# vinhsuhi/JMAC

Measured on AMD Instinct MI355X. Metric: gnn_layer_edges_per_s, higher is better.
Workload: dtype f32

## Files before the change

include/jmac_hip.h:

```cpp
#ifndef JMAC_HIP_H_
#define JMAC_HIP_H_

#include <stddef.h>
#include <stdint.h>

#ifdef __cplusplus
extern "C" {
#endif

typedef void* jmac_stream_t;

#define JMAC_OK 0
#define JMAC_EINVAL (-1)
#define JMAC_EDIM (-2)
#define JMAC_EWORKSPACE (-3)
#define JMAC_ERANGE (-4)

typedef struct { int32_t seg, beg, end, pslot; } jmac_item_t;
typedef struct { int32_t seg, pslot0, nchunks, pad; } jmac_split_t;

const char* jmac_strerror(int rc);
int jmac_version(void);


// ... 96 lines not shown

size_t jmac_bn_tanh_workspace_bytes(int64_t N, int64_t d);
int jmac_bn_tanh_fwd2_f32(const float* x, int64_t ldx, int64_t N, int64_t d, const float* weight,
                          const float* bias, float* running_mean, float* running_var,
                          int32_t training, float momentum, float eps, float* y, int64_t ldy,
                          float* y2, int64_t ldy2, float* save_mean, float* save_invstd, void* ws,
                          size_t ws_bytes, jmac_stream_t stream);
int jmac_bn_tanh_bwd2_f32(const float* x, int64_t ldx, const float* y, int64_t ldy, const float* gy,
                          int64_t ldgy, const float* gy2, int64_t ldgy2, int64_t N, int64_t d,
                          const float* weight, const float* save_mean, const float* save_invstd,
                          int32_t training, float* gx, int64_t ldgx, float* gweight, float* gbias,
                          void* ws, size_t ws_bytes, jmac_stream_t stream);

#define JMAC_BN_MAX_BLOCKS 16
size_t jmac_bn_tanh_seg_workspace_bytes(int32_t nblocks, int64_t d);
int jmac_bn_tanh_seg_fwd2_f32(const float* x, int64_t ldx, int64_t d, int32_t nblocks, const int64_t* h_blk_ptr,
                              const int32_t* h_order, const float* weight, const float* bias,
                              float* running_mean, float* running_var, float momentum, float eps, float* y,
                              int64_t ldy, float* y2, int64_t ldy2, float* save_mean, float* save_invstd,
                              void* ws, size_t ws_bytes, jmac_stream_t stream);
int jmac_bn_tanh_seg_bwd2_f32(const float* x, int64_t ldx, const float* y, int64_t ldy, const float* gy,
                              int64_t ldgy, const float* gy2, int64_t ldgy2, int64_t d, int32_t nblocks,
                              const int64_t* h_blk_ptr, const float* weight, const float* save_mean,
                              const float* save_invstd, float* gx, int64_t ldgx, float* gweight, float* gbias,
                              void* ws, size_t ws_bytes, jmac_stream_t stream);

int jmac_col_moments_f32(const float* x, int64_t ldx, int64_t N, int64_t d, float* mean, float* m2,
                         void* ws, size_t ws_bytes, jmac_stream_t stream);
int jmac_bn_tanh_apply_f32(const float* x, int64_t ldx, int64_t N, int64_t d, const float* weight,
                           const float* bias, const float* mean, const float* invstd, float* y,
                           int64_t ldy, jmac_stream_t stream);
int jmac_bn_tanh_bwd_sums_f32(const float* x, int64_t ldx, const float* y, int64_t ldy, const float* gy,
                              int64_t ldgy, int64_t N, int64_t d, const float* mean,
                              const float* invstd, float* sums, void* ws, size_t ws_bytes,
                              jmac_stream_t stream);
int jmac_bn_tanh_bwd_apply_f32(const float* x, int64_t ldx, const float* y, int64_t ldy, const float* gy,
                               int64_t ldgy, int64_t N, int64_t d, const float* weight,
                               const float* mean, const float* invstd, const float* sums,
                               int64_t n_total, float* gx, int64_t ldgx, jmac_stream_t stream);

int jmac_row_normalize_fwd_f32(const float* x, int64_t ldx, int64_t N, int64_t d, float eps, float* y,
                               int64_t ldy, float* inv, jmac_stream_t stream);
int jmac_row_normalize_bwd_f32(const float* y, int64_t ldy, const float* g, int64_t ldg, const float* inv,
                               int64_t N, int64_t d, float eps, float* gx, int64_t ldgx,
                               jmac_stream_t stream);

int jmac_row_normalize_drop_fwd_f32(const float* x, int64_t ldx, int64_t N, int64_t d, float eps,
                                    const float* mask, int64_t ldm, float scale, float* y, int64_t ldy,
                                    float* inv, jmac_stream_t stream);
int jmac_row_normalize_drop_bwd_f32(const float* x, int64_t ldx, const float* inv, const float* mask,
                                    int64_t ldm, float scale, const float* g, int64_t ldg, int64_t N,
                                    int64_t d, float eps, float* gx, int64_t ldgx, int32_t accumulate,
                                    jmac_stream_t stream);

int jmac_row_normalize_dropseed_fwd_f32(const float* x, int64_t ldx, int64_t N, int64_t d, float eps,
                                        const int64_t* seed, float p_drop, float* y, int64_t ldy,
                                        float* inv, jmac_stream_t stream);
int jmac_row_normalize_dropseed_bwd_f32(const float* x, int64_t ldx, const float* inv, const int64_t* seed,
                                        float p_drop, const float* g, int64_t ldg, int64_t N, int64_t d,
                                        float eps, float* gx, int64_t ldgx, int32_t accumulate,
                                        jmac_stream_t stream);

int jmac_rows_normalize_dropseed_fwd_f32(const float* x, int64_t ldx, const int64_t* row_map, int64_t N, int64_t d,
                                         float eps, const int64_t* seed, float p_drop, float* x_rows, int64_t ldxr,
                                         float* y, int64_t ldy, float* inv, jmac_stream_t stream);
int jmac_bn_tanh_normalize_dropseed_fwd_f32(const float* x, int64_t ldx, int64_t N, int64_t d, const float* weight,
                                            const float* bias, float* running_mean, float* running_var,
                                            int32_t training, float momentum, float eps, float* y, int64_t ldy,
                                            const int64_t* row_map, float* y_rows, int64_t ldyr, float norm_eps,
                                            const int64_t* seed, float p_drop, float* yn, int64_t ldyn, float* inv,
                                            float* save_mean, float* save_invstd, void* ws, size_t ws_bytes,
                                            jmac_stream_t stream);
int jmac_bn_tanh_bwd_normadj_f32(const float* x, int64_t ldx, const float* y, int64_t ldy, const float* inv,
                                 const float* g, int64_t ldg, float norm_eps, const int64_t* seed, float p_drop,
                                 const float* gy2, int64_t ldgy2, const int64_t* row_map, int64_t N, int64_t d,
                                 const float* weight, const float* save_mean, const float* save_invstd,
                                 int32_t training, float* gx, int64_t ldgx, float* gweight, float* gbias, void* ws,
                                 size_t ws_bytes, jmac_stream_t stream);
int jmac_row_normalize_dropseed_bwd_rows_f32(const float* x, int64_t ldx, const float* inv, const int64_t* seed,
                                             float p_drop, const float* g, int64_t ldg, const float* add,
                                             int64_t ldadd, const int64_t* row_map, int64_t N, int64_t d, float eps,
                                             float* dst, int64_t lddst, int32_t accumulate, jmac_stream_t stream);

int jmac_l1_score_f32(const float* er, int64_t lder, const float* table, int64_t ldt, int64_t B,
                      int64_t N, int64_t d, float* out, int64_t ldout, int32_t accumulate,
                      jmac_stream_t stream);
int jmac_l1_score_bf16(const uint16_t* er, int64_t lder, const uint16_t* table, int64_t ldt, int64_t B,
                       int64_t N, int64_t d, float* out, int64_t ldout, int32_t accumulate,
                       jmac_stream_t stream);

typedef struct {
    const float* ent;  int64_t ld_ent;
    const float* rel;  int64_t ld_rel;
    const void* table; int64_t ld_table;
} jmac_link_layer_t;
size_t jmac_linkpred_rank_workspace_bytes(int64_t B, int64_t d, int32_t n_layers);
int jmac_linkpred_rank_f32(const jmac_link_layer_t* layers, int32_t n_layers, const int32_t* h, const int32_t* r,
                           int32_t pred_head, const int32_t* gold, const int32_t* filt_ptr, const int32_t* filt_idx,
                           int64_t B, int64_t N, int64_t d, int32_t* rank, void* ws, size_t ws_bytes, jmac_stream_t stream);
int jmac_linkpred_rank_bf16(const jmac_link_layer_t* layers, int32_t n_layers, const int32_t* h, const int32_t* r,
                            int32_t pred_head, const int32_t* gold, const int32_t* filt_ptr, const int32_t* filt_idx,
                            int64_t B, int64_t N, int64_t d, int32_t* rank, void* ws, size_t ws_bytes, jmac_stream_t stream);

typedef struct {
    const int64_t* key;
    int64_t        n_keys;
    const int32_t* tail_ptr;
    const int32_t* tail_idx;
} jmac_tail_index_t;

int jmac_linkpred_rank_indexed_f32(const jmac_link_layer_t* layers, int32_t n_layers, const int32_t* h, const int32_t* r,
                                   int32_t pred_head, const int32_t* gold, const jmac_tail_index_t* index, int64_t B,
                                   int64_t N, int64_t d, int32_t* rank, void* ws, size_t ws_bytes, jmac_stream_t stream);
int jmac_linkpred_rank_indexed_bf16(const jmac_link_layer_t* layers, int32_t n_layers, const int32_t* h, const int32_t* r,
                                    int32_t pred_head, const int32_t* gold, const jmac_tail_index_t* index, int64_t B,
                                    int64_t N, int64_t d, int32_t* rank, void* ws, size_t ws_bytes, jmac_stream_t stream);

size_t jmac_linkpred_topk_workspace_bytes(int64_t B, int64_t N, int64_t d, int32_t n_layers, int32_t k);
int jmac_linkpred_topk_f32(const jmac_link_layer_t* layers, int32_t n_layers, const int32_t* h, const int32_t* r,
                           int32_t pred_head, const jmac_tail_index_t* index, int64_t B, int64_t N, int64_t d, int32_t k,
                           float* val, int32_t* idx, void* ws, size_t ws_bytes, jmac_stream_t stream);
int jmac_linkpred_topk_bf16(const jmac_link_layer_t* layers, int32_t n_layers, const int32_t* h, const int32_t* r,
                            int32_t pred_head, const jmac_tail_index_t* index, int64_t B, int64_t N, int64_t d, int32_t k,
                            float* val, int32_t* idx, void* ws, size_t ws_bytes, jmac_stream_t stream);

int jmac_filtered_rank_f32(const float* score, int64_t lds, const int32_t* gold,
                           const int32_t* filt_ptr, const int32_t* filt_idx, int64_t B, int64_t N,
                           int32_t descending, int32_t* rank, jmac_stream_t stream);

int jmac_sim_matrix_f32(const float* A, int64_t lda, const float* B, int64_t ldb, int64_t M,
                        int64_t N, int64_t d, float* C, int64_t ldc, jmac_stream_t stream);

size_t jmac_sim_topk_workspace_bytes(int64_t L, int64_t N, int32_t k);
int jmac_sim_topk_f32(const float* A, int64_t lda, const float* B, int64_t ldb, int64_t L, int64_t N,
                      int64_t d, int32_t k, float* val, int32_t* idx, void* ws, size_t ws_bytes,
                      jmac_stream_t stream);

int jmac_row_topk_f32(const float* S, int64_t lds, int64_t L, int64_t N, int32_t k, float* val,
                      int32_t* idx, jmac_stream_t stream);

size_t jmac_softmax_entropy_workspace_bytes(int64_t n1, int64_t n2);
int jmac_softmax_entropy_f32(const float* A, int64_t lda, const float* B, int64_t ldb, int64_t n1,
                             int64_t n2, int64_t d, float scale, float* ent_rows, float* ent_cols,
                             void* ws, size_t ws_bytes, jmac_stream_t stream);

size_t jmac_sim_softmax_stats_workspace_bytes(int64_t n1, int64_t n2);
int jmac_sim_softmax_stats_f32(const float* A, int64_t lda, const float* B, int64_t ldb, int64_t n1, int64_t n2, int64_t d,
                               float scale, float* row_max, int32_t* row_arg, float* row_sum, float* row_ent, float* col_max,
                               int32_t* col_arg, float* col_sum, float* col_ent, void* ws, size_t ws_bytes,
                               jmac_stream_t stream);

size_t jmac_sim_lse_workspace_bytes(int64_t n1, int64_t n2);
int jmac_sim_lse_f32(const float* A, int64_t lda, const float* B, int64_t ldb, int64_t n1, int64_t n2, int64_t d, float scale,
                     const float* col_add, const float* row_add, float row_shift, float col_shift, float* row_out,
                     float* col_out, void* ws, size_t ws_bytes, jmac_stream_t stream);

int jmac_row_softmax_f32(const float* S, int64_t lds, int64_t n1, int64_t n2, const uint8_t* row_mask,
                         const uint8_t* col_mask, float fill, float scale, float* out, int64_t ldo, float* ent,
                         jmac_stream_t stream);
size_t jmac_col_softmax_workspace_bytes(int64_t n1, int64_t n2);
int jmac_col_softmax_f32(const float* S, int64_t lds, int64_t n1, int64_t n2, const uint8_t* row_mask,
                         const uint8_t* col_mask, float fill, float scale, float* out_t, int64_t ldo, float* ent,
                         void* ws, size_t ws_bytes, jmac_stream_t stream);

size_t jmac_col_topk_workspace_bytes(int64_t n1, int64_t n2, int32_t k);
int jmac_col_topk_f32(const float* S, int64_t lds, int64_t n1, int64_t n2, int32_t k, float* val, void* ws,
                      size_t ws_bytes, jmac_stream_t stream);

int jmac_csls_apply_f32(const float* S, int64_t lds, int64_t n1, int64_t n2, const float* r1,
                        const float* r2, float* out, int64_t ldo, jmac_stream_t stream);

int jmac_csls_rank_f32(const float* S, int64_t lds, int64_t n1, int64_t n2, const float* r1, const float* r2,
                       const int32_t* gold, int32_t* rank, jmac_stream_t stream);

size_t jmac_sim_csls_rank_workspace_bytes(int64_t n1, int64_t n2);
int jmac_sim_csls_rank_f32(const float* A, int64_t lda, const float* B, int64_t ldb, int64_t n1, int64_t n2, int64_t d,
                           const float* r1, const float* r2, const int32_t* gold, int32_t* rank, void* ws, size_t ws_bytes,
                           jmac_stream_t stream);
size_t jmac_sim_csls_topk_workspace_bytes(int64_t n1, int64_t n2, int32_t k);
int jmac_sim_csls_topk_f32(const float* A, int64_t lda, const float* B, int64_t ldb, int64_t n1, int64_t n2, int64_t d,
                           const float* r1, const float* r2, int32_t k, float* val, int32_t* idx, void* ws, size_t ws_bytes,
                           jmac_stream_t stream);
int jmac_sim_csls_topk_viable_f32(const float* A, int64_t lda, const float* B, int64_t ldb, int64_t n1, int64_t n2, int64_t d,
                                  const float* r1, const float* r2, const int32_t* row_id, const uint64_t* best, int32_t k,
                                  float* val, int32_t* idx, void* ws, size_t ws_bytes, jmac_stream_t stream);

size_t jmac_l1_csls_topk_workspace_bytes(int64_t n1, int64_t n2, int64_t d, int32_t k);
int jmac_l1_csls_topk_f32(const float* A, int64_t lda, const float* B, int64_t ldb, int64_t n1, int64_t n2, int64_t d,
                          const float* r1, const float* r2, int32_t k, float* val, int32_t* idx, void* ws, size_t ws_bytes,
                          jmac_stream_t stream);
int jmac_l1_csls_topk_viable_f32(const float* A, int64_t lda, const float* B, int64_t ldb, int64_t n1, int64_t n2, int64_t d,
                                 const float* r1, const float* r2, const int32_t* row_id, const uint64_t* best, int32_t k,
                                 float* val, int32_t* idx, void* ws, size_t ws_bytes, jmac_stream_t stream);
size_t jmac_l1_csls_rank_workspace_bytes(int64_t n1, int64_t n2);
int jmac_l1_csls_rank_f32(const float* A, int64_t lda, const float* B, int64_t ldb, int64_t n1, int64_t n2, int64_t d,
                          const float* r1, const float* r2, const int32_t* gold, int32_t* rank, void* ws, size_t ws_bytes,
                          jmac_stream_t stream);

size_t jmac_stable_match_workspace_bytes(int64_t n1, int64_t n2);
int jmac_stable_match_f32(const int32_t* cand_idx, const float* cand_val, int64_t ld, int64_t n1, int64_t n2, int32_t k, int32_t* ptr,
                          uint64_t* best, int32_t* match1, int32_t* match2, uint64_t* counters, void* ws, size_t ws_bytes,
                          jmac_stream_t stream);

int jmac_gemm_f32(const float* A, int64_t lda, int32_t transA, const float* B, int64_t ldb,
                  int32_t transB, int64_t M, int64_t N, int64_t K, float* C, int64_t ldc,
                  jmac_stream_t stream);

#define JMAC_GEMM_MAX_TASKS 24
#define JMAC_GEMM_ACT_NONE 0
#define JMAC_GEMM_ACT_LEAKY 1
#define JMAC_GEMM_ACT_RELU 2
#define JMAC_GEMM_DACT_LEAKY 3
#define JMAC_GEMM_DACT_RELU 4
typedef struct {
    const float* A;  const float* A2;  int64_t lda;  int64_t a_split;  int32_t transA;  int32_t transB;
    const float* B;  int64_t ldb;
    float* C;  float* C2;  int64_t ldc;  int64_t c_split;
    int64_t M, N, K;
    const float* act_src;  int64_t ld_act_src;
    int32_t act;  int32_t accumulate;  float slope;  int32_t pad_;
} jmac_gemm_task_t;
int jmac_gemm_grouped_f32(const jmac_gemm_task_t* tasks, int32_t n_tasks, jmac_stream_t stream);

#define JMAC_WCAT_MAX 4
int jmac_wcat_pack_seed_f32(const float* const* w_att, const float* const* gcn, float* const* wcat, int32_t n_layers,
                            int64_t d, const float* extra_src, float* extra_dst, int64_t extra_floats,
                            int64_t* const* counters, int32_t n_counters, int64_t* seed_state, int64_t* seed_out,
                            jmac_stream_t stream);
int jmac_wcat_unpack_f32(const float* const* dwcat, float* const* d_watt, float* const* d_gcn,
                         int32_t n_layers, int64_t d, const float* extra_src, float* extra_dst,
                         int64_t extra_floats, jmac_stream_t stream);

#define JMAC_ADAM_MAX_TASKS 64
typedef struct {
    float* p;
    const float* g;
    float* m;
    float* v;
    int64_t n;
    int32_t vec4;
} jmac_adam_task_t;
int jmac_adam_step_f32(const jmac_adam_task_t* tasks, int32_t n_tasks, float* step, double* aux, double lr, double beta1,
                       double beta2, double eps, double weight_decay, int32_t decoupled, int32_t maximize, jmac_stream_t stream);

int jmac_rows_compact_f32(const float* const* h_src, const int64_t* h_ld_src, float* const* h_dst, int32_t n_tables,
                          const int64_t* idx, int64_t n_used, int64_t d, jmac_stream_t stream);
int jmac_rows_expand_f32(const float* const* h_src, float* const* h_dst, const int64_t* h_ld_dst,
                         const int32_t* h_accumulate, int32_t n_tables, const int32_t* pos, int64_t rows, int64_t d,
                         jmac_stream_t stream);


int jmac_triple_l1_fwd_f32(const float* ent, int64_t lde, const float* rel, int64_t ldr,
                           const int64_t* h, const int64_t* r, const int64_t* t, int64_t T,
                           int64_t period, int64_t d, float* score, jmac_stream_t stream);
int jmac_triple_l1_bwd_f32(const float* ent, int64_t lde, const float* rel, int64_t ldr,
                           const int64_t* h, const int64_t* r, const int64_t* t, int64_t T,
                           int64_t period, int64_t d, const float* gscore, float* dent, int64_t ldde, float* drel, int64_t lddr,
                           jmac_stream_t stream);
int jmac_pair_cosine_fwd_stats_f32(const float* e1, int64_t ld1, const float* e2, int64_t ld2, const int64_t* i1,
                                   const int64_t* i2, int64_t L, int64_t d, float* dist, float* stats,
                                   jmac_stream_t stream);
int jmac_pair_cosine_bwd_rows_f32(const float* e1, int64_t ld1, const float* e2, int64_t ld2, int64_t L, int64_t d,
                                  const float* gdist, const float* gscalar, float gscale, const float* stats,
                                  const int32_t* rec, const int32_t* rowptr, int64_t n1, int64_t n2, float* de1,
                                  int64_t ldd1, float* de2, int64_t ldd2, jmac_stream_t stream);

int jmac_triple_l1_margin_bwd_exact2_f32(const float* ent, int64_t lde, const float* rel, int64_t ldr, const int64_t* h,
                                         const int64_t* r, const int64_t* t, int64_t B, int64_t K, int64_t d,
                                         const float* score, const float* gamma, const float* gloss, int64_t ent_off,
                                         int64_t rel_off, float* cnt_ent, float* cnt_rel, float* dent, int64_t rows_ent,
                                         int32_t acc_ent, float* drel, int64_t rows_rel, int32_t acc_rel,
                                         jmac_stream_t stream);

int jmac_triple_l1_margin_fwd_counts_f32(const float* ent, int64_t lde, const float* rel, int64_t ldr, const int64_t* h,
                                         const int64_t* r, const int64_t* t, int64_t B, int64_t K, int64_t d,
                                         const float* gamma, int64_t ent_off, int64_t rel_off, float* cnt_ent,
                                         float* cnt_rel, float* score, jmac_stream_t stream);
int jmac_margin_counts_scale_clear_f32(float* cnt_ent, float* cnt_rel, const float* gloss, int64_t B, int64_t K, int64_t d,
                                       float* dent, int64_t rows_ent, int32_t acc_ent, float* drel, int64_t rows_rel,
                                       int32_t acc_rel, jmac_stream_t stream);

int jmac_vec_mean_acc_f32(const float* x, int64_t n, const float* add_to, float* out, jmac_stream_t stream);

int jmac_pair_cosine_fwd_f32(const float* e1, int64_t ld1, const float* e2, int64_t ld2,
                             const int64_t* i1, const int64_t* i2, int64_t L, int64_t d, float* dist,
                             jmac_stream_t stream);
int jmac_pair_cosine_bwd_f32(const float* e1, int64_t ld1, const float* e2, int64_t ld2,
                             const int64_t* i1, const int64_t* i2, int64_t L, int64_t d,
                             const float* gdist, float* de1, int64_t ldd1, float* de2, int64_t ldd2,
                             jmac_stream_t stream);

int jmac_margin_loss_fwd_acc_f32(const float* score, int64_t B, int64_t K, const float* gamma, const float* add_to,
                                 float* loss, jmac_stream_t stream);
int jmac_margin_loss_bwd_f32(const float* score, int64_t B, int64_t K, const float* gamma,
                             const float* gloss, float* dscore, jmac_stream_t stream);


int jmac_sample_completion_batch(const int64_t* triples, int64_t T, const int64_t* perm, const int32_t* key_of_triple,
                                 const int32_t* tail_ptr, const int32_t* tail_idx, int64_t num_ent, int64_t B, int64_t K,
                                 const int64_t* seed, int64_t* step, int64_t* batch_h, int64_t* batch_r, int64_t* batch_t,
                                 jmac_stream_t stream);

int jmac_scatter_sum_f32(const float* src, const int64_t* index, int64_t E, int64_t d, int64_t N,
                         float* out, jmac_stream_t stream);
size_t jmac_scatter_softmax_workspace_bytes(int64_t N, int64_t d);
int jmac_scatter_softmax_f32(const float* src, const int64_t* index, int64_t E, int64_t d, int64_t N,
                             float* out, void* ws, size_t ws_bytes, jmac_stream_t stream);

#ifdef __cplusplus
}
#endif
#endif
```

jmac_amd/_lib.py:

```python
from __future__ import annotations

import ctypes as C
import os
import re
import weakref
from typing import Optional

_HERE = os.path.dirname(os.path.abspath(__file__))
LIB_PATH = os.environ.get("JMAC_LIB_PATH") or os.path.join(_HERE, "libjmac_hip.so")
HEADER_PATH = os.path.join(os.path.dirname(_HERE), "include", "jmac_hip.h")

_lib: Optional[C.CDLL] = None

i32, i64, f32, vp, sz = C.c_int32, C.c_int64, C.c_float, C.c_void_p, C.c_size_t


class JmacError(RuntimeError):
    pass


class View(C.Structure):
    _fields_ = [("ptr", vp), ("order", vp), ("items", vp), ("splits", vp), ("counts", vp),
                ("n_items_max", i64), ("n_splits_max", i64), ("n_parts_max", i64),
                ("item_edges", vp), ("n_empty", i64), ("n_coop", i64), ("entry_dst", vp)]


class LinkLayer(C.Structure):
    _fields_ = [("ent", vp), ("ld_ent", i64), ("rel", vp), ("ld_rel", i64), ("table", vp), ("ld_table", i64)]


class TailIndex(C.Structure):
    _fields_ = [("key", vp), ("n_keys", i64), ("tail_ptr", vp), ("tail_idx", vp)]


class AggFwdJob(C.Structure):
    _fields_ = [("P", vp), ("ldp", i64), ("QZ", vp), ("ldqz", i64), ("RR", vp), ("ldrr", i64), ("a_att", vp), ("col", vp), ("etype", vp),
                ("by_dst", C.POINTER(View)), ("N", i64), ("d", i64), ("slope", f32), ("loop_rel", i32), ("self_off", i64),
                ("out_scale", f32), ("out", vp), ("ldo", i64), ("seg_max", vp), ("seg_den", vp), ("ws", vp), ("ws_bytes", sz)]


class AdamTask(C.Structure):
    _fields_ = [("p", vp), ("g", vp), ("m", vp), ("v", vp), ("n", i64), ("vec4", i32)]


class GemmTask(C.Structure):
    _fields_ = [("A", vp), ("A2", vp), ("lda", i64), ("a_split", i64), ("transA", i32), ("transB", i32),
                ("B", vp), ("ldb", i64), ("C", vp), ("C2", vp), ("ldc", i64), ("c_split", i64),
                ("M", i64), ("N", i64), ("K", i64), ("act_src", vp), ("ld_act_src", i64),
                ("act", i32), ("accumulate", i32), ("slope", f32), ("pad_", i32)]


_SIGS = {
    "jmac_strerror": (C.c_char_p, [C.c_int]),
    "jmac_version": (C.c_int, []),
    "jmac_graph_workspace_bytes": (sz, [i64, i64]),
    "jmac_index_check": (C.c_int, [vp, i32, i64, i64, i64, vp, vp]),
    "jmac_csr_build": (C.c_int, [vp, vp, i64, i64, i64, vp, vp, vp, vp, vp, sz, vp]),
    "jmac_group_build": (C.c_int, [vp, i64, i64, vp, vp, vp, sz, vp]),
    "jmac_items_max": (i64, [i64, i64, i32, i32]),
    "jmac_splits_max": (i64, [i64, i32, i32]),
    "jmac_parts_max": (i64, [i64, i32, i32]),
    "jmac_items_build": (C.c_int, [vp, i64, i32, i32, i32, vp, vp, vp, vp, sz, vp]),
    "jmac_rel_attn_fwd_workspace_bytes": (sz, [i64, i64]),
    "jmac_item_edges_build": (C.c_int, [vp, vp, i64, vp, vp, vp, vp]),
    "jmac_rel_attn_aggregate_fwd_f32": (C.c_int, [vp, i64, vp, i64, vp, i64, vp, vp, vp, C.POINTER(View),
                                                  i64, i64, f32, i32, i64, f32, vp, i64, vp, vp, vp, sz, vp]),
    "jmac_rel_attn_aggregate_fwd_bf16": (C.c_int, [vp, i64, vp, i64, vp, i64, vp, vp, vp, C.POINTER(View),
                                                   i64, i64, f32, i32, i64, f32, vp, i64, vp, vp, vp, sz, vp]),
    "jmac_rel_attn_aggregate_fwd_bf16_padded": (C.c_int, [vp, i64, vp, i64, vp, i64, i64, vp, vp, vp, C.POINTER(View),
                                                          i64, i64, f32, i32, i64, f32, vp, i64, vp, vp, vp, sz, vp]),
    "jmac_rel_attn_aggregate_fwd_jobs_f32": (C.c_int, [C.POINTER(AggFwdJob), i32, vp]),
    "jmac_softmax_parts_merge_f32": (C.c_int, [vp, i64, vp, vp, vp, i32, i64, i64, vp, i64, vp, f32, vp, i64, vp, vp, vp]),
    "jmac_rel_attn_bwd_workspace_bytes": (sz, [i64, i64, i64, i64, i64, i64, i64, i32]),
    "jmac_rel_attn_aggregate_bwd_f32": (C.c_int, [vp, i64, vp, i64, vp, i64, vp, vp, vp, vp,
                                                  C.POINTER(View), C.POINTER(View), C.POINTER(View),
                                                  i64, i64, i64, i64, i64, f32, i32, i64, f32, vp, i64, vp, vp, vp, i64,
                                                  vp, i64, vp, i64, vp, i64, vp, i32, vp, sz, vp]),
    "jmac_rel_attn_aggregate_bwd_phases_f32": (C.c_int, [vp, i64, vp, i64, vp, i64, vp, vp, vp, vp,
                                                         C.POINTER(View), C.POINTER(View), C.POINTER(View),
                                                         i64, i64, i64, i64, i64, f32, i32, i64, f32, vp, i64, vp, vp, vp, i64,
                                                         vp, i64, vp, i64, vp, i64, vp, i32, vp, sz, vp]),
    "jmac_bn_tanh_workspace_bytes": (sz, [i64, i64]),
    "jmac_bn_tanh_fwd2_f32": (C.c_int, [vp, i64, i64, i64, vp, vp, vp, vp, i32, f32, f32, vp, i64, vp, i64, vp, vp,
                                        vp, sz, vp]),
    "jmac_bn_tanh_bwd2_f32": (C.c_int, [vp, i64, vp, i64, vp, i64, vp, i64, i64, i64, vp, vp, vp, i32, vp, i64, vp, vp,
                                        vp, sz, vp]),
    "jmac_bn_tanh_seg_workspace_bytes": (sz, [i32, i64]),
    "jmac_bn_tanh_seg_fwd2_f32": (C.c_int, [vp, i64, i64, i32, C.POINTER(i64), C.POINTER(i32), vp, vp, vp, vp, f32, f32, vp, i64,
                                            vp, i64, vp, vp, vp, sz, vp]),
    "jmac_bn_tanh_seg_bwd2_f32": (C.c_int, [vp, i64, vp, i64, vp, i64, vp, i64, i64, i32, C.POINTER(i64), vp, vp, vp, vp, i64,
                                            vp, vp, vp, sz, vp]),
    "jmac_row_normalize_drop_fwd_f32": (C.c_int, [vp, i64, i64, i64, f32, vp, i64, f32, vp, i64, vp, vp]),
    "jmac_row_normalize_drop_bwd_f32": (C.c_int, [vp, i64, vp, vp, i64, f32, vp, i64, i64, i64, f32, vp, i64, i32, vp]),
    "jmac_row_normalize_dropseed_fwd_f32": (C.c_int, [vp, i64, i64, i64, f32, vp, f32, vp, i64, vp, vp]),
    "jmac_row_normalize_dropseed_bwd_f32": (C.c_int, [vp, i64, vp, vp, f32, vp, i64, i64, i64, f32, vp, i64, i32, vp]),
    "jmac_rows_normalize_dropseed_fwd_f32": (C.c_int, [vp, i64, vp, i64, i64, f32, vp, f32, vp, i64, vp, i64, vp, vp]),
    "jmac_bn_tanh_normalize_dropseed_fwd_f32": (C.c_int, [vp, i64, i64, i64, vp, vp, vp, vp, i32, f32, f32, vp, i64, vp, vp, i64,
                                                          f32, vp, f32, vp, i64, vp, vp, vp, vp, sz, vp]),
    "jmac_bn_tanh_bwd_normadj_f32": (C.c_int, [vp, i64, vp, i64, vp, vp, i64, f32, vp, f32, vp, i64, vp, i64, i64, vp, vp, vp,
                                               i32, vp, i64, vp, vp, vp, sz, vp]),
    "jmac_row_normalize_dropseed_bwd_rows_f32": (C.c_int, [vp, i64, vp, vp, f32, vp, i64, vp, i64, vp, i64, i64, f32, vp, i64,
                                                           i32, vp]),
    "jmac_gemm_grouped_f32": (C.c_int, [C.POINTER(GemmTask), i32, vp]),
    "jmac_wcat_pack_seed_f32": (C.c_int, [C.POINTER(vp), C.POINTER(vp), C.POINTER(vp), i32, i64, vp, vp, i64, C.POINTER(vp), i32, vp, vp, vp]),
    "jmac_adam_step_f32": (C.c_int, [C.POINTER(AdamTask), i32, vp, vp, C.c_double, C.c_double, C.c_double, C.c_double, C.c_double, i32, i32,
                                     vp]),
    "jmac_wcat_unpack_f32": (C.c_int, [C.POINTER(vp), C.POINTER(vp), C.POINTER(vp), i32, i64, vp, vp, i64, vp]),
    "jmac_rows_compact_f32": (C.c_int, [C.POINTER(vp), C.POINTER(i64), C.POINTER(vp), i32, vp, i64, i64, vp]),
    "jmac_rows_expand_f32": (C.c_int, [C.POINTER(vp), C.POINTER(vp), C.POINTER(i64), C.POINTER(i32), i32, vp, i64, i64, vp]),
    "jmac_col_moments_f32": (C.c_int, [vp, i64, i64, i64, vp, vp, vp, sz, vp]),
    "jmac_bn_tanh_apply_f32": (C.c_int, [vp, i64, i64, i64, vp, vp, vp, vp, vp, i64, vp]),
    "jmac_bn_tanh_bwd_sums_f32": (C.c_int, [vp, i64, vp, i64, vp, i64, i64, i64, vp, vp, vp, vp, sz, vp]),
    "jmac_bn_tanh_bwd_apply_f32": (C.c_int, [vp, i64, vp, i64, vp, i64, i64, i64, vp, vp, vp, vp, i64, vp, i64, vp]),
    "jmac_row_normalize_fwd_f32": (C.c_int, [vp, i64, i64, i64, f32, vp, i64, vp, vp]),
    "jmac_row_normalize_bwd_f32": (C.c_int, [vp, i64, vp, i64, vp, i64, i64, f32, vp, i64, vp]),
    "jmac_l1_score_f32": (C.c_int, [vp, i64, vp, i64, i64, i64, i64, vp, i64, i32, vp]),
    "jmac_l1_score_bf16": (C.c_int, [vp, i64, vp, i64, i64, i64, i64, vp, i64, i32, vp]),
    "jmac_filtered_rank_f32": (C.c_int, [vp, i64, vp, vp, vp, i64, i64, i32, vp, vp]),
    "jmac_linkpred_rank_workspace_bytes": (sz, [i64, i64, i32]),
    "jmac_linkpred_rank_f32": (C.c_int, [vp, i32, vp, vp, i32, vp, vp, vp, i64, i64, i64, vp, vp, sz, vp]),
    "jmac_linkpred_rank_bf16": (C.c_int, [vp, i32, vp, vp, i32, vp, vp, vp, i64, i64, i64, vp, vp, sz, vp]),
    "jmac_linkpred_rank_indexed_f32": (C.c_int, [vp, i32, vp, vp, i32, vp, vp, i64, i64, i64, vp, vp, sz, vp]),
    "jmac_linkpred_rank_indexed_bf16": (C.c_int, [vp, i32, vp, vp, i32, vp, vp, i64, i64, i64, vp, vp, sz, vp]),
    "jmac_linkpred_topk_workspace_bytes": (sz, [i64, i64, i64, i32, i32]),
    "jmac_linkpred_topk_f32": (C.c_int, [vp, i32, vp, vp, i32, vp, i64, i64, i64, i32, vp, vp, vp, sz, vp]),
    "jmac_linkpred_topk_bf16": (C.c_int, [vp, i32, vp, vp, i32, vp, i64, i64, i64, i32, vp, vp, vp, sz, vp]),
    "jmac_sim_matrix_f32": (C.c_int, [vp, i64, vp, i64, i64, i64, i64, vp, i64, vp]),
    "jmac_sim_topk_workspace_bytes": (sz, [i64, i64, i32]),
    "jmac_sim_topk_f32": (C.c_int, [vp, i64, vp, i64, i64, i64, i64, i32, vp, vp, vp, sz, vp]),
    "jmac_col_topk_workspace_bytes": (sz, [i64, i64, i32]),
    "jmac_col_topk_f32": (C.c_int, [vp, i64, i64, i64, i32, vp, vp, sz, vp]),
    "jmac_row_topk_f32": (C.c_int, [vp, i64, i64, i64, i32, vp, vp, vp]),
    "jmac_softmax_entropy_workspace_bytes": (sz, [i64, i64]),
    "jmac_softmax_entropy_f32": (C.c_int, [vp, i64, vp, i64, i64, i64, i64, f32, vp, vp, vp, sz, vp]),
    "jmac_sim_softmax_stats_workspace_bytes": (sz, [i64, i64]),
    "jmac_sim_softmax_stats_f32": (C.c_int, [vp, i64, vp, i64, i64, i64, i64, f32, vp, vp, vp, vp, vp, vp, vp, vp, vp, sz, vp]),
    "jmac_sim_lse_workspace_bytes": (sz, [i64, i64]),
    "jmac_sim_lse_f32": (C.c_int, [vp, i64, vp, i64, i64, i64, i64, f32, vp, vp, f32, f32, vp, vp, vp, sz, vp]),
    "jmac_row_softmax_f32": (C.c_int, [vp, i64, i64, i64, vp, vp, f32, f32, vp, i64, vp, vp]),
    "jmac_col_softmax_workspace_bytes": (sz, [i64, i64]),
    "jmac_col_softmax_f32": (C.c_int, [vp, i64, i64, i64, vp, vp, f32, f32, vp, i64, vp, vp, sz, vp]),
    "jmac_csls_rank_f32": (C.c_int, [vp, i64, i64, i64, vp, vp, vp, vp, vp]),
    "jmac_csls_apply_f32": (C.c_int, [vp, i64, i64, i64, vp, vp, vp, i64, vp]),
    "jmac_sim_csls_rank_workspace_bytes": (sz, [i64, i64]),
    "jmac_sim_csls_rank_f32": (C.c_int, [vp, i64, vp, i64, i64, i64, i64, vp, vp, vp, vp, vp, sz, vp]),
    "jmac_sim_csls_topk_workspace_bytes": (sz, [i64, i64, i32]),
    "jmac_sim_csls_topk_f32": (C.c_int, [vp, i64, vp, i64, i64, i64, i64, vp, vp, i32, vp, vp, vp, sz, vp]),
    "jmac_sim_csls_topk_viable_f32": (C.c_int, [vp, i64, vp, i64, i64, i64, i64, vp, vp, vp, vp, i32, vp, vp, vp, sz, vp]),
    "jmac_l1_csls_topk_workspace_bytes": (sz, [i64, i64, i64, i32]),
    "jmac_l1_csls_topk_f32": (C.c_int, [vp, i64, vp, i64, i64, i64, i64, vp, vp, i32, vp, vp, vp, sz, vp]),
    "jmac_l1_csls_topk_viable_f32": (C.c_int, [vp, i64, vp, i64, i64, i64, i64, vp, vp, vp, vp, i32, vp, vp, vp, sz, vp]),
    "jmac_l1_csls_rank_workspace_bytes": (sz, [i64, i64]),
    "jmac_l1_csls_rank_f32": (C.c_int, [vp, i64, vp, i64, i64, i64, i64, vp, vp, vp, vp, vp, sz, vp]),
    "jmac_stable_match_workspace_bytes": (sz, [i64, i64]),
    "jmac_stable_match_f32": (C.c_int, [vp, vp, i64, i64, i64, i32, vp, vp, vp, vp, vp, vp, sz, vp]),
    "jmac_gemm_f32": (C.c_int, [vp, i64, i32, vp, i64, i32, i64, i64, i64, vp, i64, vp]),
    "jmac_triple_l1_fwd_f32": (C.c_int, [vp, i64, vp, i64, vp, vp, vp, i64, i64, i64, vp, vp]),
    "jmac_triple_l1_bwd_f32": (C.c_int, [vp, i64, vp, i64, vp, vp, vp, i64, i64, i64, vp, vp, i64, vp, i64, vp]),
    "jmac_pair_cosine_fwd_stats_f32": (C.c_int, [vp, i64, vp, i64, vp, vp, i64, i64, vp, vp, vp]),
    "jmac_pair_cosine_fwd_f32": (C.c_int, [vp, i64, vp, i64, vp, vp, i64, i64, vp, vp]),
    "jmac_pair_cosine_bwd_f32": (C.c_int, [vp, i64, vp, i64, vp, vp, i64, i64, vp, vp, i64, vp, i64, vp]),
    "jmac_pair_cosine_bwd_rows_f32": (C.c_int, [vp, i64, vp, i64, i64, i64, vp, vp, f32, vp, vp, vp, i64, i64, vp, i64, vp, i64, vp]),
    "jmac_triple_l1_margin_bwd_exact2_f32": (C.c_int, [vp, i64, vp, i64, vp, vp, vp, i64, i64, i64, vp, vp, vp, i64, i64, vp, vp,
                                                       vp, i64, i32, vp, i64, i32, vp]),
    "jmac_triple_l1_margin_fwd_counts_f32": (C.c_int, [vp, i64, vp, i64, vp, vp, vp, i64, i64, i64, vp, i64, i64, vp, vp, vp, vp]),
    "jmac_margin_counts_scale_clear_f32": (C.c_int, [vp, vp, vp, i64, i64, i64, vp, i64, i32, vp, i64, i32, vp]),
    "jmac_vec_mean_acc_f32": (C.c_int, [vp, i64, vp, vp, vp]),
    "jmac_margin_loss_fwd_acc_f32": (C.c_int, [vp, i64, i64, vp, vp, vp, vp]),
    "jmac_margin_loss_bwd_f32": (C.c_int, [vp, i64, i64, vp, vp, vp, vp]),
    "jmac_sample_completion_batch": (C.c_int, [vp, i64, vp, vp, vp, vp, i64, i64, i64, vp, vp, vp, vp, vp, vp]),
    "jmac_scatter_sum_f32": (C.c_int, [vp, vp, i64, i64, i64, vp, vp]),
    "jmac_scatter_softmax_workspace_bytes": (sz, [i64, i64]),
    "jmac_scatter_softmax_f32": (C.c_int, [vp, vp, i64, i64, i64, vp, vp, sz, vp]),
}


_TESTING_SIGS = {
    "jmac_rel_attn_aggregate_fwd_lanes64_f32": _SIGS["jmac_rel_attn_aggregate_fwd_f32"],
    "jmac_rel_attn_aggregate_fwd_lanes64_bf16_padded": _SIGS["jmac_rel_attn_aggregate_fwd_bf16_padded"],
    "jmac_gemm_nt_x3_f32": (C.c_int, [vp, i64, vp, i64, i64, i64, i64, vp, i64, vp]),
}


def header_text(path: str = HEADER_PATH) -> str:
    return re.sub(r"/\*.*?\*/", "", open(path).read(), flags=re.S)


# ... 122 lines not shown
```

jmac_amd/csrc/norm.hip:

```cpp
#include <initializer_list>

#include "common.h"

using namespace jmac;

namespace {

constexpr int kBlock = 256;
constexpr int kStatBlocks = 512;

__global__ __launch_bounds__(kBlock) void col_stats_partial_kernel(const float* __restrict__ x, int64_t ldx, int64_t N,
                                                                   int D4, float* __restrict__ partial) {
    extern __shared__ __attribute__((aligned(16))) char smem[];
    float4* red = reinterpret_cast<float4*>(smem);
    const int rpb = kBlock / D4 > 0 ? kBlock / D4 : 1;
    const int tid = threadIdx.x;
    for (int cbase = 0; cbase < D4; cbase += kBlock) {
        const int rsub = D4 >= kBlock ? 0 : tid / D4;
        const int c4 = D4 >= kBlock ? cbase + tid : tid % D4;
        const bool active = (D4 >= kBlock ? c4 < D4 : tid < rpb * D4);
        float4 s1 = f4zero(), s2 = f4zero();
        if (active) {
            const float4 K = ld4(x + c4 * 4);
            for (int64_t r = (int64_t)blockIdx.x * rpb + rsub; r < N; r += (int64_t)gridDim.x * rpb) {
                float4 v = ld4(x + r * ldx + c4 * 4);
                v.x -= K.x; v.y -= K.y; v.z -= K.z; v.w -= K.w;
                s1.x += v.x; s1.y += v.y; s1.z += v.z; s1.w += v.w;
                s2.x = fmaf(v.x, v.x, s2.x); s2.y = fmaf(v.y, v.y, s2.y); s2.z = fmaf(v.z, v.z, s2.z); s2.w = fmaf(v.w, v.w, s2.w);
            }
        }
        if (D4 >= kBlock) {
            if (active) {
                st4(partial + ((int64_t)blockIdx.x * 2 + 0) * D4 * 4 + c4 * 4, s1);
                st4(partial + ((int64_t)blockIdx.x * 2 + 1) * D4 * 4 + c4 * 4, s2);
            }
        } else {
            if (active) {
                red[(0 * rpb + rsub) * D4 + c4] = s1;
                red[(1 * rpb + rsub) * D4 + c4] = s2;
            }
            __syncthreads();
            if (tid < D4) {
                float4 a1 = red[tid], a2 = red[rpb * D4 + tid];
                for (int q = 1; q < rpb; ++q) {
                    float4 b1 = red[q * D4 + tid], b2 = red[(rpb + q) * D4 + tid];
                    a1.x += b1.x; a1.y += b1.y; a1.z += b1.z; a1.w += b1.w;
                    a2.x += b2.x; a2.y += b2.y; a2.z += b2.z; a2.w += b2.w;
                }
                st4(partial + ((int64_t)blockIdx.x * 2 + 0) * D4 * 4 + tid * 4, a1);
                st4(partial + ((int64_t)blockIdx.x * 2 + 1) * D4 * 4 + tid * 4, a2);
            }
            break;
        }
    }
}

__global__ void bn_finalize_kernel(const float* __restrict__ sums, const float* __restrict__ x, int64_t N,
                                   int d, float eps, float momentum, float* __restrict__ running_mean,
                                   float* __restrict__ running_var, float* __restrict__ save_mean,
                                   float* __restrict__ save_invstd) {
    const int c = blockIdx.x * blockDim.x + threadIdx.x;
    if (c >= d) return;
    const float s1 = sums[c], s2 = sums[d + c];
    const float n = (float)N;
    const float K = x[c];
    const float mshift = s1 / n;
    const float mean = K + mshift;
    float var = s2 / n - mshift * mshift;
    var = var > 0.f ? var : 0.f;
    save_mean[c] = mean;
    save_invstd[c] = rsqrtf(var + eps);
    if (running_mean) running_mean[c] = (1.f - momentum) * running_mean[c] + momentum * mean;
    if (running_var) {
        const float unbiased = N > 1 ? var * n / (n - 1.f) : var;
        running_var[c] = (1.f - momentum) * running_var[c] + momentum * unbiased;
    }
}

constexpr int RF_COLS = 16, RF_LANES = 1024 / RF_COLS;
__global__ __launch_bounds__(1024) void bn_reduce_finalize_kernel(const float* __restrict__ partial, int nparts,
                                                                  const float* __restrict__ x, int64_t N, int d, float eps,
                                                                  float momentum, float* __restrict__ running_mean,
                                                                  float* __restrict__ running_var, float* __restrict__ save_mean,
                                                                  float* __restrict__ save_invstd) {
    __shared__ float red1[RF_LANES][RF_COLS], red2[RF_LANES][RF_COLS];
    const int cl = threadIdx.x % RF_COLS, rl = threadIdx.x / RF_COLS;
    const int c = blockIdx.x * RF_COLS + cl;
    float a1 = 0.f, a2 = 0.f, b1 = 0.f, b2 = 0.f;
    if (c < d) {
        int p = rl;
        for (; p + RF_LANES < nparts; p += 2 * RF_LANES) {
            a1 += partial[(int64_t)p * 2 * d + c];
            a2 += partial[(int64_t)p * 2 * d + d + c];
            b1 += partial[(int64_t)(p + RF_LANES) * 2 * d + c];
            b2 += partial[(int64_t)(p + RF_LANES) * 2 * d + d + c];
        }
        if (p < nparts) {
            a1 += partial[(int64_t)p * 2 * d + c];
            a2 += partial[(int64_t)p * 2 * d + d + c];
        }
    }
    red1[rl][cl] = a1 + b1;
    red2[rl][cl] = a2 + b2;
    __syncthreads();
    if (rl == 0 && c < d) {
        float s1 = red1[0][cl], s2 = red2[0][cl];
#pragma unroll 8
        for (int r = 1; r < RF_LANES; ++r) {
            s1 += red1[r][cl];
            s2 += red2[r][cl];
        }
        const float n = (float)N;
        const float mshift = s1 / n;
        const float mean = x[c] + mshift;
        float var = s2 / n - mshift * mshift;
        var = var > 0.f ? var : 0.f;
        save_mean[c] = mean;
        save_invstd[c] = rsqrtf(var + eps);
        if (running_mean) running_mean[c] = (1.f - momentum) * running_mean[c] + momentum * mean;
        if (running_var) {
            const float unbiased = N > 1 ? var * n / (n - 1.f) : var;
            running_var[c] = (1.f - momentum) * running_var[c] + momentum * unbiased;
        }
    }
}

__global__ void moments_finalize_kernel(const float* __restrict__ sums, const float* __restrict__ x, int64_t N, int d,
                                        float* __restrict__ mean, float* __restrict__ m2) {
    const int c = blockIdx.x * blockDim.x + threadIdx.x;
    if (c >= d) return;
    const float s1 = sums[c], s2 = sums[d + c], n = (float)N;
    mean[c] = x[c] + s1 / n;
    const float v = s2 - s1 * s1 / n;
    m2[c] = v > 0.f ? v : 0.f;
}

__global__ void bn_eval_stats_kernel(const float* __restrict__ running_mean, const float* __restrict__ running_var, int d,
                                     float eps, float* __restrict__ save_mean, float* __restrict__ save_invstd) {
    const int c = blockIdx.x * blockDim.x + threadIdx.x;
    if (c < d) {
        save_mean[c] = running_mean[c];
        save_invstd[c] = rsqrtf(running_var[c] + eps);
    }
}

__global__ __launch_bounds__(kBlock) void bn_tanh_apply_kernel(const float* __restrict__ x, int64_t ldx, int64_t N, int D4,
                                                               const float* __restrict__ weight, const float* __restrict__ bias,
                                                               const float* __restrict__ mean, const float* __restrict__ invstd,
                                                               float* __restrict__ y, int64_t ldy, float* __restrict__ y2,
                                                               int64_t ldy2) {
    const int64_t total = N * D4;
    for (int64_t i = (int64_t)blockIdx.x * kBlock + threadIdx.x; i < total; i += (int64_t)gridDim.x * kBlock) {
        const int64_t r = i / D4;
        const int c4 = (int)(i % D4);
        const float4 v = ld4(x + r * ldx + c4 * 4);
        const float4 mu = ld4(mean + c4 * 4), is = ld4(invstd + c4 * 4), w = ld4(weight + c4 * 4), b = ld4(bias + c4 * 4);
        float4 o;
        o.x = tanhf(fmaf((v.x - mu.x) * is.x, w.x, b.x));
        o.y = tanhf(fmaf((v.y - mu.y) * is.y, w.y, b.y));
        o.z = tanhf(fmaf((v.z - mu.z) * is.z, w.z, b.z));
        o.w = tanhf(fmaf((v.w - mu.w) * is.w, w.w, b.w));
        st4(y + r * ldy + c4 * 4, o);
        if (y2) st4(y2 + r * ldy2 + c4 * 4, o);
    }
}

__global__ __launch_bounds__(kBlock) void bn_bwd_partial_kernel(const float* __restrict__ x, int64_t ldx,
                                                                const float* __restrict__ y, int64_t ldy,
                                                                const float* __restrict__ gy, int64_t ldgy,
                                                                const float* __restrict__ gy2, int64_t ldgy2, int64_t N, int D4,
                                                                const float* __restrict__ mean, const float* __restrict__ invstd,
                                                                float* __restrict__ partial) {
    extern __shared__ __attribute__((aligned(16))) char smem[];
    float4* red = reinterpret_cast<float4*>(smem);
    const int rpb = kBlock / D4 > 0 ? kBlock / D4 : 1;
    const int tid = threadIdx.x;
    for (int cbase = 0; cbase < D4; cbase += kBlock) {
        const int rsub = D4 >= kBlock ? 0 : tid / D4;
        const int c4 = D4 >= kBlock ? cbase + tid : tid % D4;
        const bool active = (D4 >= kBlock ? c4 < D4 : tid < rpb * D4);
        float4 s1 = f4zero(), s2 = f4zero();
        if (active) {
            const float4 mu = ld4(mean + c4 * 4), is = ld4(invstd + c4 * 4);
            for (int64_t r = (int64_t)blockIdx.x * rpb + rsub; r < N; r += (int64_t)gridDim.x * rpb) {
                const float4 xv = ld4(x + r * ldx + c4 * 4), yv = ld4(y + r * ldy + c4 * 4);
                float4 g = ld4(gy + r * ldgy + c4 * 4);
                if (gy2) {
                    const float4 g2 = ld4(gy2 + r * ldgy2 + c4 * 4);
                    g.x += g2.x; g.y += g2.y; g.z += g2.z; g.w += g2.w;
                }
                const float gz0 = g.x * (1.f - yv.x * yv.x), gz1 = g.y * (1.f - yv.y * yv.y);
                const float gz2 = g.z * (1.f - yv.z * yv.z), gz3 = g.w * (1.f - yv.w * yv.w);
                s1.x += gz0; s1.y += gz1; s1.z += gz2; s1.w += gz3;
                s2.x = fmaf(gz0, (xv.x - mu.x) * is.x, s2.x); s2.y = fmaf(gz1, (xv.y - mu.y) * is.y, s2.y);
                s2.z = fmaf(gz2, (xv.z - mu.z) * is.z, s2.z); s2.w = fmaf(gz3, (xv.w - mu.w) * is.w, s2.w);
            }
        }
        if (D4 >= kBlock) {
            if (active) {
                st4(partial + ((int64_t)blockIdx.x * 2 + 0) * D4 * 4 + c4 * 4, s1);
                st4(partial + ((int64_t)blockIdx.x * 2 + 1) * D4 * 4 + c4 * 4, s2);
            }
        } else {
            if (active) {
                red[(0 * rpb + rsub) * D4 + c4] = s1;
                red[(1 * rpb + rsub) * D4 + c4] = s2;
            }
// ... 940 lines not shown
#pragma unroll
            for (int k = 0; k < 2; ++k) {
                const int c = (ok[k] ? cc[k] : 0) * 4;
                xv[u][k] = ld4(x + row[u] * ldx + c);
                yv[u][k] = ld4(y + row[u] * ldy + c);
                q[u][k] = ld4(g + row[u] * ldg + c);
                if (gy2) g2[u][k] = ld4(gy2 + s[u] * ldgy2 + c);
            }
        }
        normalize_drop_adjoint_rows<SEED, ROWFORM, R>(ds, key, row, D4, cc, ok, eps, iv, yv, q);
#pragma unroll
        for (int u = 0; u < R; ++u) {
            if (r0 + u >= N) break;
#pragma unroll
            for (int k = 0; k < 2; ++k) {
                if (!ok[k]) continue;
                float4 gg = adjoint_scale(iv[u], q[u][k]);
                if (gy2) gg = add4(gg, g2[u][k]);
                const float4 yy = yv[u][k], xx = xv[u][k];
                float4 o;
#define JMAC_BN_BWD(comp)                                                                                                       \
                o.comp = bn_bwd_apply_elem(gg.comp, yy.comp, xx.comp, mu[k].comp, is[k].comp, w[k].comp, gw[k].comp, gb[k].comp, \
                                           training, invn);
                JMAC_BN_BWD(x) JMAC_BN_BWD(y) JMAC_BN_BWD(z) JMAC_BN_BWD(w)
#undef JMAC_BN_BWD
                st4(gx + (r0 + u) * ldgx + cc[k] * 4, o);
            }
        }
    }
}

template <bool SEED, bool ROWFORM, int R>
__global__ __launch_bounds__(kBlock) void row_normalize_drop_bwd_scatter_kernel(const float* __restrict__ x, int64_t ldx,
                                                                                const float* __restrict__ inv, DropSrc ds,
                                                                                const float* __restrict__ g, int64_t ldg,
                                                                                const float* __restrict__ add, int64_t ldadd,
                                                                                const int64_t* __restrict__ map, int64_t N, int D4,
                                                                                float eps, float* __restrict__ dst, int64_t lddst,
                                                                                int accumulate) {
    const int lane = lane_id();
    const int64_t w0 = (int64_t)blockIdx.x * (kBlock / 64) + (threadIdx.x >> 6), nw = (int64_t)gridDim.x * (kBlock / 64);
    const uint2 key = drop_key(ds, SEED);
    const int cc[2] = {lane, lane + 64};
    const bool ok[2] = {cc[0] < D4, cc[1] < D4};
    for (int64_t r0 = w0 * R; r0 < N; r0 += nw * R) {
        float4 v[R][2], q[R][2], p[R][2], old[R][2];
        float iv[R];
        int64_t row[R], s[R];
#pragma unroll
        for (int u = 0; u < R; ++u) {
            row[u] = r0 + u < N ? r0 + u : N - 1;
            s[u] = map ? map[row[u]] : row[u];
        }
#pragma unroll
        for (int u = 0; u < R; ++u) {
            iv[u] = inv[row[u]];
#pragma unroll
            for (int k = 0; k < 2; ++k) {
                const int c = (ok[k] ? cc[k] : 0) * 4;
                v[u][k] = ld4(x + row[u] * ldx + c);
                q[u][k] = ld4(g + row[u] * ldg + c);
                if (add) p[u][k] = ld4(add + row[u] * ldadd + c);
                if (accumulate) old[u][k] = ld4(dst + s[u] * lddst + c);
            }
        }
        normalize_drop_adjoint_rows<SEED, ROWFORM, R>(ds, key, row, D4, cc, ok, eps, iv, v, q);
#pragma unroll
        for (int u = 0; u < R; ++u) {
            if (r0 + u >= N) break;
#pragma unroll
            for (int k = 0; k < 2; ++k) {
                if (!ok[k]) continue;
                float4 o = add ? adjoint_scale_add<ROWFORM>(iv[u], q[u][k], p[u][k]) : adjoint_scale(iv[u], q[u][k]);
                if (accumulate) o = add4(o, old[u][k]);
                st4(dst + s[u] * lddst + cc[k] * 4, o);
            }
        }
    }
}

constexpr int kDropRows = 4;
constexpr int64_t kDropRowsMinN = 2048;

}

extern "C" {

size_t jmac_bn_tanh_workspace_bytes(int64_t N, int64_t d) {
    (void)N;
    return align_up((size_t)(kStatBlocks + 1) * 2 * (d > 0 ? d : 0) * 4) + 256;
}

int jmac_bn_tanh_fwd2_f32(const float* x, int64_t ldx, int64_t N, int64_t d, const float* weight, const float* bias,
                          float* running_mean, float* running_var, int32_t training, float momentum, float eps, float* y,
                          int64_t ldy, float* y2, int64_t ldy2, float* save_mean, float* save_invstd, void* ws, size_t ws_bytes,
                          jmac_stream_t stream) {
    if (N < 0 || !weight || !bias || !save_mean || !save_invstd) return JMAC_EINVAL;
    if (d <= 0 || d % 4 || ldx % 4 || ldy % 4 || (y2 && ldy2 % 4)) return JMAC_EDIM;
    if (N == 0) return JMAC_OK;
    if (!x || !y) return JMAC_EINVAL;
    hipStream_t st = (hipStream_t)stream;
    const int D4 = (int)(d / 4);
    if (training) {
        if (!ws || ws_bytes < jmac_bn_tanh_workspace_bytes(N, d)) return JMAC_EWORKSPACE;
        float* partial = (float*)ws;
        const unsigned g = stat_grid(N, D4);
        hipLaunchKernelGGL(col_stats_partial_kernel, dim3(g), dim3(kBlock), stat_smem(D4), st, x, ldx, N, D4, partial);
        hipLaunchKernelGGL(bn_reduce_finalize_kernel, dim3((unsigned)((d + RF_COLS - 1) / RF_COLS)), dim3(1024), 0, st, partial,
                           (int)g, x, N, (int)d, eps, momentum, running_mean, running_var, save_mean, save_invstd);
    } else {
        if (!running_mean || !running_var) return JMAC_EINVAL;
        hipLaunchKernelGGL(bn_eval_stats_kernel, dim3((unsigned)((d + 255) / 256)), dim3(256), 0, st, running_mean, running_var,
                           (int)d, eps, save_mean, save_invstd);
    }
    hipLaunchKernelGGL(bn_tanh_apply_kernel, dim3(stream_grid(N * D4)), dim3(kBlock), 0, st, x, ldx, N, D4, weight, bias,
                       save_mean, save_invstd, y, ldy, y2, ldy2);
    return (int)hipGetLastError();
}

int jmac_bn_tanh_bwd2_f32(const float* x, int64_t ldx, const float* y, int64_t ldy, const float* gy, int64_t ldgy,
                          const float* gy2, int64_t ldgy2, int64_t N, int64_t d, const float* weight, const float* save_mean,
                          const float* save_invstd, int32_t training, float* gx, int64_t ldgx, float* gweight, float* gbias,
                          void* ws, size_t ws_bytes, jmac_stream_t stream) {
    if (N < 0 || !weight || !save_mean || !save_invstd || !gweight || !gbias) return JMAC_EINVAL;
    if (d <= 0 || d % 4 || ldx % 4 || ldy % 4 || ldgy % 4 || ldgx % 4 || (gy2 && ldgy2 % 4)) return JMAC_EDIM;
    if (!ws || ws_bytes < jmac_bn_tanh_workspace_bytes(N, d)) return JMAC_EWORKSPACE;
    hipStream_t st = (hipStream_t)stream;
    const int D4 = (int)(d / 4);
    float* partial = (float*)ws;
    unsigned g = 0;
    if (N > 0) {
        if (!x || !y || !gy || !gx) return JMAC_EINVAL;
        g = stat_grid(N, D4);
        hipLaunchKernelGGL(bn_bwd_partial_kernel, dim3(g), dim3(kBlock), stat_smem(D4), st, x, ldx, y, ldy, gy, ldgy, gy2, ldgy2, N,
                           D4, save_mean, save_invstd, partial);
    }
    if (gweight == gbias + d) {
        launch_reduce_rows(partial, (int)g, (int)(2 * d), 1.f, gbias, st);
    } else {
        float* sums = partial + (size_t)kStatBlocks * 2 * d;
        launch_reduce_rows(partial, (int)g, (int)(2 * d), 1.f, sums, st);
        hipLaunchKernelGGL(bn_bwd_finalize_kernel, dim3((unsigned)((d + 255) / 256)), dim3(256), 0, st, sums, (int)d, gweight, gbias);
    }
    if (N > 0)
        hipLaunchKernelGGL(bn_bwd_apply_kernel, dim3(stream_grid(N * D4)), dim3(kBlock), 0, st, x, ldx, y, ldy, gy, ldgy, gy2, ldgy2, N,
                           D4, weight, save_mean, save_invstd, gweight, gbias, training, 1.f / (float)N, gx, ldgx);
    return (int)hipGetLastError();
}

int jmac_row_normalize_fwd_f32(const float* x, int64_t ldx, int64_t N, int64_t d, float eps, float* y, int64_t ldy, float* inv,
                               jmac_stream_t stream) {
    if (N < 0 || d <= 0 || d >= INT32_MAX) return JMAC_EINVAL;
    if (N == 0) return JMAC_OK;
    if (!x || !y || !inv) return JMAC_EINVAL;
    int64_t blocks = (N + kBlock / 64 - 1) / (kBlock / 64);
    if (blocks > 8192) blocks = 8192;
    hipLaunchKernelGGL(row_normalize_fwd_kernel, dim3((unsigned)blocks), dim3(kBlock), 0, (hipStream_t)stream, x, ldx, N, (int)d, eps,
                       y, ldy, inv);
    return (int)hipGetLastError();
}

int jmac_row_normalize_bwd_f32(const float* y, int64_t ldy, const float* g, int64_t ldg, const float* inv, int64_t N, int64_t d,
                               float eps, float* gx, int64_t ldgx, jmac_stream_t stream) {
    if (N < 0 || d <= 0 || d >= INT32_MAX) return JMAC_EINVAL;
    if (N == 0) return JMAC_OK;
    if (!y || !g || !inv || !gx) return JMAC_EINVAL;
    int64_t blocks = (N + kBlock / 64 - 1) / (kBlock / 64);
    if (blocks > 8192) blocks = 8192;
    hipLaunchKernelGGL(row_normalize_bwd_kernel, dim3((unsigned)blocks), dim3(kBlock), 0, (hipStream_t)stream, y, ldy, g, ldg, inv, N,
                       (int)d, eps, gx, ldgx);
    return (int)hipGetLastError();
}

static int drop_fwd(const float* x, int64_t ldx, int64_t N, int64_t d, float eps, const DropSrc& ds, bool seeded, float* y, int64_t ldy,
                    float* inv, jmac_stream_t stream) {
    if (N < 0 || d <= 0 || d >= INT32_MAX) return JMAC_EINVAL;
    if (d % 4 || ldx % 4 || ldy % 4 || (ds.mask && ds.ldm % 4)) return JMAC_EDIM;
    if (N == 0) return JMAC_OK;
    if (!x || !y || !inv) return JMAC_EINVAL;
    if ((((uintptr_t)x | (uintptr_t)y | (uintptr_t)ds.mask) & 15) != 0) return JMAC_EDIM;
    if (d <= 512 && N >= kDropRowsMinN) {
        int64_t rb = ((N + kDropRows - 1) / kDropRows + kBlock / 64 - 1) / (kBlock / 64);
        if (rb > 8192) rb = 8192;
        if (seeded)
            hipLaunchKernelGGL((row_normalize_drop_fwd_rows_kernel<true, kDropRows>), dim3((unsigned)rb), dim3(kBlock), 0,
                               (hipStream_t)stream, x, ldx, N, (int)(d / 4), eps, ds, y, ldy, inv);
        else
            hipLaunchKernelGGL((row_normalize_drop_fwd_rows_kernel<false, kDropRows>), dim3((unsigned)rb), dim3(kBlock), 0,
                               (hipStream_t)stream, x, ldx, N, (int)(d / 4), eps, ds, y, ldy, inv);
        return (int)hipGetLastError();
    }
    int64_t blocks = (N + kBlock / 64 - 1) / (kBlock / 64);
    if (blocks > 8192) blocks = 8192;
    if (seeded)
        hipLaunchKernelGGL(row_normalize_drop_fwd_kernel<true>, dim3((unsigned)blocks), dim3(kBlock), 0, (hipStream_t)stream, x, ldx, N,
                           (int)(d / 4), eps, ds, y, ldy, inv);
    else
        hipLaunchKernelGGL(row_normalize_drop_fwd_kernel<false>, dim3((unsigned)blocks), dim3(kBlock), 0, (hipStream_t)stream, x, ldx, N,
                           (int)(d / 4), eps, ds, y, ldy, inv);
    return (int)hipGetLastError();
}

static int drop_bwd(const float* x, int64_t ldx, const float* inv, const DropSrc& ds, bool seeded, const float* g, int64_t ldg, int64_t N,
                    int64_t d, float eps, float* gx, int64_t ldgx, int32_t accumulate, jmac_stream_t stream) {
    if (N < 0 || d <= 0 || d >= INT32_MAX) return JMAC_EINVAL;
    if (d % 4 || ldx % 4 || ldg % 4 || ldgx % 4 || (ds.mask && ds.ldm % 4)) return JMAC_EDIM;
    if (N == 0) return JMAC_OK;
    if (!x || !inv || !g || !gx) return JMAC_EINVAL;
    if ((((uintptr_t)x | (uintptr_t)g | (uintptr_t)gx | (uintptr_t)ds.mask) & 15) != 0) return JMAC_EDIM;
    if (d <= 512 && N >= kDropRowsMinN) {
        int64_t rb = ((N + kDropRows - 1) / kDropRows + kBlock / 64 - 1) / (kBlock / 64);
        if (rb > 8192) rb = 8192;
        if (seeded)
            hipLaunchKernelGGL((row_normalize_drop_bwd_rows_kernel<true, kDropRows>), dim3((unsigned)rb), dim3(kBlock), 0,
                               (hipStream_t)stream, x, ldx, inv, ds, g, ldg, N, (int)(d / 4), eps, gx, ldgx, accumulate ? 1 : 0);
        else
            hipLaunchKernelGGL((row_normalize_drop_bwd_rows_kernel<false, kDropRows>), dim3((unsigned)rb), dim3(kBlock), 0,
                               (hipStream_t)stream, x, ldx, inv, ds, g, ldg, N, (int)(d / 4), eps, gx, ldgx, accumulate ? 1 : 0);
        return (int)hipGetLastError();
    }
    int64_t blocks = (N + kBlock / 64 - 1) / (kBlock / 64);
    if (blocks > 8192) blocks = 8192;
    if (seeded)
        hipLaunchKernelGGL(row_normalize_drop_bwd_kernel<true>, dim3((unsigned)blocks), dim3(kBlock), 0, (hipStream_t)stream, x, ldx, inv,
                           ds, g, ldg, N, (int)(d / 4), eps, gx, ldgx, accumulate ? 1 : 0);
    else
        hipLaunchKernelGGL(row_normalize_drop_bwd_kernel<false>, dim3((unsigned)blocks), dim3(kBlock), 0, (hipStream_t)stream, x, ldx, inv,
                           ds, g, ldg, N, (int)(d / 4), eps, gx, ldgx, accumulate ? 1 : 0);
    return (int)hipGetLastError();
}

static int seeded_src(const int64_t* seed, float p_drop, DropSrc& ds) {
    if (!seed || !(p_drop >= 0.f) || !(p_drop < 1.f)) return JMAC_EINVAL;
    const double keep = 1.0 - (double)p_drop, t = keep * 4294967296.0;
    ds = DropSrc{nullptr, 0, seed, t >= 4294967295.0 ? 0xFFFFFFFFu : (uint32_t)t, (float)(1.0 / keep)};
    return JMAC_OK;
}

int jmac_row_normalize_drop_fwd_f32(const float* x, int64_t ldx, int64_t N, int64_t d, float eps, const float* mask, int64_t ldm,
                                    float scale, float* y, int64_t ldy, float* inv, jmac_stream_t stream) {
    return drop_fwd(x, ldx, N, d, eps, DropSrc{mask, ldm, nullptr, 0u, scale}, false, y, ldy, inv, stream);
}

int jmac_row_normalize_drop_bwd_f32(const float* x, int64_t ldx, const float* inv, const float* mask, int64_t ldm, float scale,
                                    const float* g, int64_t ldg, int64_t N, int64_t d, float eps, float* gx, int64_t ldgx,
                                    int32_t accumulate, jmac_stream_t stream) {
    return drop_bwd(x, ldx, inv, DropSrc{mask, ldm, nullptr, 0u, scale}, false, g, ldg, N, d, eps, gx, ldgx, accumulate, stream);
}

int jmac_row_normalize_dropseed_fwd_f32(const float* x, int64_t ldx, int64_t N, int64_t d, float eps, const int64_t* seed,
                                        float p_drop, float* y, int64_t ldy, float* inv, jmac_stream_t stream) {
    DropSrc ds;
    if (int rc = seeded_src(seed, p_drop, ds)) return rc;
    return drop_fwd(x, ldx, N, d, eps, ds, true, y, ldy, inv, stream);
}

int jmac_row_normalize_dropseed_bwd_f32(const float* x, int64_t ldx, const float* inv, const int64_t* seed, float p_drop,
                                        const float* g, int64_t ldg, int64_t N, int64_t d, float eps, float* gx, int64_t ldgx,
                                        int32_t accumulate, jmac_stream_t stream) {
    DropSrc ds;
    if (int rc = seeded_src(seed, p_drop, ds)) return rc;
    return drop_bwd(x, ldx, inv, ds, true, g, ldg, N, d, eps, gx, ldgx, accumulate, stream);
}

static int fused_src(const int64_t* seed, float p_drop, DropSrc& ds) {
    if (seed) return seeded_src(seed, p_drop, ds);
    ds = DropSrc{nullptr, 0, nullptr, 0u, 1.f};
    return JMAC_OK;
}
static bool aligned16(std::initializer_list<const void*> ps) {
    uintptr_t a = 0;
    for (const void* p : ps) a |= (uintptr_t)p;
    return (a & 15) == 0;
}
static unsigned rows_grid(int64_t N, int R) {
    int64_t rb = ((N + R - 1) / R + kBlock / 64 - 1) / (kBlock / 64);
    return (unsigned)(rb > 8192 ? 8192 : rb);
}
#define JMAC_LAUNCH_SEEDED(kernel, R, grid, st, ...)                                                                      \
    do {                                                                                                                  \
        if (ds.seed) hipLaunchKernelGGL((kernel<true, R>), dim3(grid), dim3(kBlock), 0, st, __VA_ARGS__);                 \
        else hipLaunchKernelGGL((kernel<false, R>), dim3(grid), dim3(kBlock), 0, st, __VA_ARGS__);                        \
    } while (0)
#define JMAC_LAUNCH_ADJ(kernel, R, grid, st, ...)                                                                         \
    do {                                                                                                                  \
        const bool rowform = N >= kDropRowsMinN;                                                                          \
        if (ds.seed && rowform) hipLaunchKernelGGL((kernel<true, true, R>), dim3(grid), dim3(kBlock), 0, st, __VA_ARGS__); \
        else if (ds.seed) hipLaunchKernelGGL((kernel<true, false, R>), dim3(grid), dim3(kBlock), 0, st, __VA_ARGS__);     \
        else if (rowform) hipLaunchKernelGGL((kernel<false, true, R>), dim3(grid), dim3(kBlock), 0, st, __VA_ARGS__);     \
        else hipLaunchKernelGGL((kernel<false, false, R>), dim3(grid), dim3(kBlock), 0, st, __VA_ARGS__);                 \
    } while (0)

int jmac_rows_normalize_dropseed_fwd_f32(const float* x, int64_t ldx, const int64_t* row_map, int64_t N, int64_t d, float eps,
                                         const int64_t* seed, float p_drop, float* x_rows, int64_t ldxr, float* y, int64_t ldy,
                                         float* inv, jmac_stream_t stream) {
    DropSrc ds;
    if (int rc = fused_src(seed, p_drop, ds)) return rc;
    if (N < 0) return JMAC_EINVAL;
    if (d <= 0 || d > 512 || d % 4 || ldx % 4 || ldy % 4 || (x_rows && ldxr % 4)) return JMAC_EDIM;
    if (N == 0) return JMAC_OK;
    if (!x || !y || !inv) return JMAC_EINVAL;
    if (!aligned16({x, y, x_rows})) return JMAC_EDIM;
    JMAC_LAUNCH_SEEDED(rows_normalize_drop_fwd_kernel, kFuseRows, rows_grid(N, kFuseRows), (hipStream_t)stream, x, ldx, row_map, N,
                       (int)(d / 4), eps, ds, x_rows, ldxr, y, ldy, inv);
    return (int)hipGetLastError();
}

int jmac_bn_tanh_normalize_dropseed_fwd_f32(const float* x, int64_t ldx, int64_t N, int64_t d, const float* weight, const float* bias,
                                            float* running_mean, float* running_var, int32_t training, float momentum, float eps,
                                            float* y, int64_t ldy, const int64_t* row_map, float* y_rows, int64_t ldyr, float norm_eps,
                                            const int64_t* seed, float p_drop, float* yn, int64_t ldyn, float* inv, float* save_mean,
                                            float* save_invstd, void* ws, size_t ws_bytes, jmac_stream_t stream) {
    DropSrc ds;
    if (int rc = fused_src(seed, p_drop, ds)) return rc;
    if (N < 0 || !weight || !bias || !save_mean || !save_invstd || (row_map == nullptr) != (y_rows == nullptr)) return JMAC_EINVAL;
    if (d <= 0 || d > 512 || d % 4 || ldx % 4 || ldy % 4 || ldyn % 4 || (y_rows && ldyr % 4)) return JMAC_EDIM;
    if (N == 0) return JMAC_OK;
    if (!x || !y || !yn || !inv) return JMAC_EINVAL;
    if (!aligned16({x, y, y_rows, yn, weight, bias, save_mean, save_invstd})) return JMAC_EDIM;
    hipStream_t st = (hipStream_t)stream;
    const int D4 = (int)(d / 4);
    if (training) {
        if (!ws || ws_bytes < jmac_bn_tanh_workspace_bytes(N, d)) return JMAC_EWORKSPACE;
        float* partial = (float*)ws;
        const unsigned g = stat_grid(N, D4);
        hipLaunchKernelGGL(col_stats_partial_kernel, dim3(g), dim3(kBlock), stat_smem(D4), st, x, ldx, N, D4, partial);
        hipLaunchKernelGGL(bn_reduce_finalize_kernel, dim3((unsigned)((d + RF_COLS - 1) / RF_COLS)), dim3(1024), 0, st, partial,
                           (int)g, x, N, (int)d, eps, momentum, running_mean, running_var, save_mean, save_invstd);
    } else {
        if (!running_mean || !running_var) return JMAC_EINVAL;
        hipLaunchKernelGGL(bn_eval_stats_kernel, dim3((unsigned)((d + 255) / 256)), dim3(256), 0, st, running_mean, running_var,
                           (int)d, eps, save_mean, save_invstd);
    }
    JMAC_LAUNCH_SEEDED(bn_tanh_normalize_drop_fwd_kernel, kFuseRows, rows_grid(N, kFuseRows), st, x, ldx, N, D4, weight, bias,
                       (const float*)save_mean, (const float*)save_invstd, y, ldy, row_map, y_rows, ldyr, norm_eps, ds, yn, ldyn, inv);
    return (int)hipGetLastError();
}

int jmac_bn_tanh_bwd_normadj_f32(const float* x, int64_t ldx, const float* y, int64_t ldy, const float* inv, const float* g,
                                 int64_t ldg, float norm_eps, const int64_t* seed, float p_drop, const float* gy2, int64_t ldgy2,
                                 const int64_t* row_map, int64_t N, int64_t d, const float* weight, const float* save_mean,
                                 const float* save_invstd, int32_t training, float* gx, int64_t ldgx, float* gweight, float* gbias,
                                 void* ws, size_t ws_bytes, jmac_stream_t stream) {
    DropSrc ds;
    if (int rc = fused_src(seed, p_drop, ds)) return rc;
    if (N < 0 || !weight || !save_mean || !save_invstd || !gweight || !gbias) return JMAC_EINVAL;
    if (d <= 0 || d > 512 || d % 4 || ldx % 4 || ldy % 4 || ldg % 4 || ldgx % 4 || (gy2 && ldgy2 % 4)) return JMAC_EDIM;
    if (!ws || ws_bytes < jmac_bn_tanh_workspace_bytes(N, d)) return JMAC_EWORKSPACE;
    if (!aligned16({x, y, g, gy2, gx, weight, save_mean, save_invstd, gweight, gbias, ws})) return JMAC_EDIM;
    hipStream_t st = (hipStream_t)stream;
    const int D4 = (int)(d / 4);
    float* partial = (float*)ws;
    unsigned pg = 0;
    if (N > 0) {
        if (!x || !y || !inv || !g || !gx) return JMAC_EINVAL;
        pg = stat_grid(N, D4);
        const int rpb = kBlock / D4;
        const unsigned threads = 64u * (unsigned)(rpb < kBlock / 64 ? rpb : kBlock / 64);
        const bool rowform = N >= kDropRowsMinN;
#define JMAC_PARTIAL(SD, RF)                                                                                                      \
        hipLaunchKernelGGL((bn_bwd_partial_adj_kernel<SD, RF, kFuseBwdRows>), dim3(pg), dim3(threads), stat_smem(D4), st, x, ldx, \
                           y, ldy, g, ldg, inv, ds, norm_eps, gy2, ldgy2, row_map, N, D4, save_mean, save_invstd, partial)
        if (ds.seed && rowform) JMAC_PARTIAL(true, true);
        else if (ds.seed) JMAC_PARTIAL(true, false);
        else if (rowform) JMAC_PARTIAL(false, true);
        else JMAC_PARTIAL(false, false);
#undef JMAC_PARTIAL
    }
    if (gweight == gbias + d) {
        launch_reduce_rows(partial, (int)pg, (int)(2 * d), 1.f, gbias, st);
    } else {
        float* sums = partial + (size_t)kStatBlocks * 2 * d;
        launch_reduce_rows(partial, (int)pg, (int)(2 * d), 1.f, sums, st);
        hipLaunchKernelGGL(bn_bwd_finalize_kernel, dim3((unsigned)((d + 255) / 256)), dim3(256), 0, st, sums, (int)d, gweight, gbias);
    }
    if (N > 0)
        JMAC_LAUNCH_ADJ(bn_bwd_apply_adj_kernel, kFuseBwdRows, rows_grid(N, kFuseBwdRows), st, x, ldx, y, ldy, g, ldg, inv, ds,
                           norm_eps, gy2, ldgy2, row_map, N, D4, weight, save_mean, save_invstd, (const float*)gweight,
                           (const float*)gbias, training ? 1 : 0, 1.f / (float)N, gx, ldgx);
    return (int)hipGetLastError();
}

int jmac_row_normalize_dropseed_bwd_rows_f32(const float* x, int64_t ldx, const float* inv, const int64_t* seed, float p_drop,
                                             const float* g, int64_t ldg, const float* add, int64_t ldadd, const int64_t* row_map,
                                             int64_t N, int64_t d, float eps, float* dst, int64_t lddst, int32_t accumulate,
                                             jmac_stream_t stream) {
    DropSrc ds;
    if (int rc = fused_src(seed, p_drop, ds)) return rc;
    if (N < 0) return JMAC_EINVAL;
    if (d <= 0 || d > 512 || d % 4 || ldx % 4 || ldg % 4 || lddst % 4 || (add && ldadd % 4)) return JMAC_EDIM;
    if (N == 0) return JMAC_OK;
    if (!x || !inv || !g || !dst) return JMAC_EINVAL;
    if (!aligned16({x, g, add, dst})) return JMAC_EDIM;
    JMAC_LAUNCH_ADJ(row_normalize_drop_bwd_scatter_kernel, kFuseBwdRows, rows_grid(N, kFuseBwdRows), (hipStream_t)stream, x, ldx,
                       inv, ds, g, ldg, add, ldadd, row_map, N, (int)(d / 4), eps, dst, lddst, accumulate ? 1 : 0);
    return (int)hipGetLastError();
}
#undef JMAC_LAUNCH_SEEDED
#undef JMAC_LAUNCH_ADJ

static int make_seg(int32_t nblocks, const int64_t* blk_ptr, const int32_t* order, int D4, SegTab& s) {
    if (nblocks < 1 || nblocks > kMaxSeg || !blk_ptr || blk_ptr[0] != 0) return JMAC_EINVAL;
    s.nb = nblocks;
    unsigned seen = 0;
    s.gofs[0] = 0;
    for (int b = 0; b < kMaxSeg; ++b) s.order[b] = 0;
    for (int b = 0; b < nblocks; ++b) {
        const int64_t n = blk_ptr[b + 1] - blk_ptr[b];
        if (n <= 0) return JMAC_EINVAL;
        s.ptr[b] = blk_ptr[b];
        s.gofs[b + 1] = s.gofs[b] + (int)stat_grid(n, D4);
        const int o = order ? order[b] : b;
        if (o < 0 || o >= nblocks || (seen >> o & 1u)) return JMAC_EINVAL;
        seen |= 1u << o;
        s.order[b] = o;
    }
    for (int b = nblocks; b <= kMaxSeg; ++b) s.ptr[b] = blk_ptr[nblocks];
    for (int b = nblocks + 1; b <= kMaxSeg; ++b) s.gofs[b] = s.gofs[nblocks];
    return JMAC_OK;
// ... 116 lines not shown
```

jmac_amd/csrc/optim.hip:

```cpp
#include "common.h"

namespace {

constexpr int kAdamBlock = 256;

struct AdamArgs {
    jmac_adam_task_t t[JMAC_ADAM_MAX_TASKS];
    int chunk_end[JMAC_ADAM_MAX_TASKS];
    int n_tasks, n_chunks;
    double lr, beta1, beta2, eps, weight_decay;
    int decoupled, maximize, advance;
    float* step;
    double* aux;
};

struct AdamConst {
    float one_minus_b1, b2, one_minus_b2, step_size, inv_bc2_sqrt, eps, wd, lr_wd;
};

__device__ __forceinline__ void adam_elem(float& p, float g, float& m, float& v, const AdamConst& c, bool decoupled, bool maximize) {
    if (maximize) g = -g;
    if (c.wd != 0.f) {
        if (decoupled) p = p - c.lr_wd * p;
        else g = g + c.wd * p;
    }
    m = m + (g - m) * c.one_minus_b1;
    v = v * c.b2 + c.one_minus_b2 * g * g;
    const float denom = __fsqrt_rn(v) * c.inv_bc2_sqrt + c.eps;
    p = p - c.step_size * (m / denom);
}

template <int V>
__global__ __launch_bounds__(kAdamBlock) void adam_step_kernel(const AdamArgs a) {
    constexpr int kChunk = kAdamBlock * 4 * V;
    const int ch = blockIdx.x;
    int task = 0;
    if (a.n_chunks > 0) {
        int lo = 0, hi = a.n_tasks - 1;
        while (lo < hi) {
            const int mid = (lo + hi) >> 1;
            if (ch >= a.chunk_end[mid]) lo = mid + 1; else hi = mid;
        }
        task = lo;
    }
    const jmac_adam_task_t T = a.t[task];
    const int first = task ? a.chunk_end[task - 1] : 0;
    const int64_t base = (int64_t)(ch - first) * kChunk;
    const int64_t left = a.n_chunks > 0 ? T.n - base : 0;
    const bool full = left >= kChunk && T.vec4;
    float4 p[V], g[V], m[V], v[V];
    if (full) {
        const float4* p4 = reinterpret_cast<const float4*>(T.p + base);
        const float4* g4 = reinterpret_cast<const float4*>(T.g + base);
        const float4* m4 = reinterpret_cast<const float4*>(T.m + base);
        const float4* v4 = reinterpret_cast<const float4*>(T.v + base);
#pragma unroll
        for (int u = 0; u < V; ++u) {
            const int i = threadIdx.x + u * kAdamBlock;
            p[u] = p4[i]; g[u] = g4[i]; m[u] = m4[i]; v[u] = v4[i];
        }
    }
    AdamConst c;
    {
        const double bc1 = 1.0 - a.aux[0] * a.beta1, bc2 = 1.0 - a.aux[1] * a.beta2;
        c.one_minus_b1 = (float)(1.0 - a.beta1);
        c.b2 = (float)a.beta2;
        c.one_minus_b2 = (float)(1.0 - a.beta2);
        c.step_size = (float)(a.lr / bc1);
        c.inv_bc2_sqrt = (float)(1.0 / sqrt(bc2));
        c.eps = (float)a.eps;
        c.wd = (float)a.weight_decay;
        c.lr_wd = (float)(a.lr * a.weight_decay);
    }
    const bool dec = a.decoupled != 0, mx = a.maximize != 0;
    if (full) {
        float4* p4 = reinterpret_cast<float4*>(T.p + base);
        float4* m4 = reinterpret_cast<float4*>(T.m + base);
        float4* v4 = reinterpret_cast<float4*>(T.v + base);
#pragma unroll
        for (int u = 0; u < V; ++u) {
            adam_elem(p[u].x, g[u].x, m[u].x, v[u].x, c, dec, mx);
            adam_elem(p[u].y, g[u].y, m[u].y, v[u].y, c, dec, mx);
            adam_elem(p[u].z, g[u].z, m[u].z, v[u].z, c, dec, mx);
            adam_elem(p[u].w, g[u].w, m[u].w, v[u].w, c, dec, mx);
        }
#pragma unroll
        for (int u = 0; u < V; ++u) {
            const int i = threadIdx.x + u * kAdamBlock;
            p4[i] = p[u]; m4[i] = m[u]; v4[i] = v[u];
        }
    } else {
        const int64_t n = left < kChunk ? left : kChunk;
        for (int64_t i = threadIdx.x; i < n; i += kAdamBlock) {
            float pp = T.p[base + i], mm = T.m[base + i], vv = T.v[base + i];
            adam_elem(pp, T.g[base + i], mm, vv, c, dec, mx);
            T.p[base + i] = pp; T.m[base + i] = mm; T.v[base + i] = vv;
        }
    }
    if (a.advance) {
        __syncthreads();
        if (threadIdx.x == 0) {
            unsigned int* ticket = reinterpret_cast<unsigned int*>(a.aux + 2);
            const unsigned int done = __hip_atomic_fetch_add(ticket, 1u, __ATOMIC_RELAXED, __HIP_MEMORY_SCOPE_AGENT);
            if (done == gridDim.x - 1) {
                a.step[0] = a.step[0] + 1.f;
                a.aux[0] = a.aux[0] * a.beta1;
                a.aux[1] = a.aux[1] * a.beta2;
                __hip_atomic_store(ticket, 0u, __ATOMIC_RELAXED, __HIP_MEMORY_SCOPE_AGENT);
            }
        }
    }
}

template <int V>
int launch_adam(const jmac_adam_task_t* tasks, int32_t n_tasks, float* step, double* aux, double lr, double beta1, double beta2,
                double eps, double weight_decay, int32_t decoupled, int32_t maximize, hipStream_t st) {
    constexpr int kChunk = kAdamBlock * 4 * V;
    int32_t at = 0;
    do {
        AdamArgs a;
        const int32_t n = (n_tasks - at) < JMAC_ADAM_MAX_TASKS ? (n_tasks - at) : JMAC_ADAM_MAX_TASKS;
        int64_t chunks = 0;
        for (int32_t i = 0; i < n; ++i) {
            const jmac_adam_task_t& t = tasks[at + i];
            if (t.n < 0 || (t.n > 0 && (!t.p || !t.g || !t.m || !t.v))) return JMAC_EINVAL;
            a.t[i] = t;
            a.t[i].vec4 = !(((uintptr_t)t.p | (uintptr_t)t.g | (uintptr_t)t.m | (uintptr_t)t.v) & 15);
            chunks += (t.n + kChunk - 1) / kChunk;
            if (chunks >= INT32_MAX) return JMAC_ERANGE;
            a.chunk_end[i] = (int)chunks;
        }
        for (int32_t i = n; i < JMAC_ADAM_MAX_TASKS; ++i) {
            a.t[i] = jmac_adam_task_t{nullptr, nullptr, nullptr, nullptr, 0, 0};
            a.chunk_end[i] = INT32_MAX;
        }
        a.n_tasks = n > 0 ? n : 1;
        a.n_chunks = (int)chunks;
        a.lr = lr; a.beta1 = beta1; a.beta2 = beta2; a.eps = eps; a.weight_decay = weight_decay;
        a.decoupled = decoupled; a.maximize = maximize;
        at += n;
        a.advance = at >= n_tasks;
        a.step = step;
        a.aux = aux;
        hipLaunchKernelGGL(adam_step_kernel<V>, dim3((unsigned)(chunks < 1 ? 1 : chunks)), dim3(kAdamBlock), 0, st, a);
        const int rc = (int)hipGetLastError();
        if (rc) return rc;
    } while (at < n_tasks);
    return JMAC_OK;
}

}

extern "C" int jmac_adam_step_f32(const jmac_adam_task_t* tasks, int32_t n_tasks, float* step, double* aux, double lr, double beta1,
                                  double beta2, double eps, double weight_decay, int32_t decoupled, int32_t maximize,
                                  jmac_stream_t stream) {
    if (n_tasks < 0 || !step || !aux || ((uintptr_t)aux & 7) || (n_tasks > 0 && !tasks)) return JMAC_EINVAL;
    if (!(lr >= 0.0) || !(eps >= 0.0) || !(beta1 >= 0.0 && beta1 < 1.0) || !(beta2 >= 0.0 && beta2 < 1.0) || !(weight_decay >= 0.0))
        return JMAC_EINVAL;
    for (int32_t i = 0; i < n_tasks; ++i)
        if (tasks[i].n < 0 || (tasks[i].n > 0 && (!tasks[i].p || !tasks[i].g || !tasks[i].m || !tasks[i].v))) return JMAC_EINVAL;
    return launch_adam<4>(tasks, n_tasks, step, aux, lr, beta1, beta2, eps, weight_decay, decoupled, maximize, (hipStream_t)stream);
}
```

jmac_amd/csrc/scatter.hip:

```cpp
#include "common.h"

using namespace jmac;

namespace {

__device__ __forceinline__ void atomic_max_f32(float* addr, float v) {
    if (v >= 0.f) atomicMax(reinterpret_cast<int*>(addr), __float_as_int(v));
    else atomicMin(reinterpret_cast<unsigned int*>(addr), __float_as_uint(v));
}

__global__ void scatter_sum_kernel(const float* __restrict__ src, const int64_t* __restrict__ index, int64_t E, int64_t d,
                                   int64_t N, float* __restrict__ out) {
    const int64_t total = E * d;
    for (int64_t i = (int64_t)blockIdx.x * blockDim.x + threadIdx.x; i < total; i += (int64_t)gridDim.x * blockDim.x) {
        const int64_t e = i / d, c = i % d;
        const int64_t r = index[e];
        if (r >= 0 && r < N) atomicAdd(out + r * d + c, src[i]);
    }
}

__global__ void fill_f32_kernel(float* __restrict__ p, int64_t n, float v) {
    for (int64_t i = (int64_t)blockIdx.x * blockDim.x + threadIdx.x; i < n; i += (int64_t)gridDim.x * blockDim.x) p[i] = v;
}

// ... 5 lines not shown
        const int64_t r = index[e];
        if (r >= 0 && r < N) atomic_max_f32(mx + r * d + c, src[i]);
    }
}

__global__ void seg_expsum_kernel(const float* __restrict__ src, const int64_t* __restrict__ index, int64_t E, int64_t d,
                                  int64_t N, const float* __restrict__ mx, float* __restrict__ sum, float* __restrict__ out) {
    const int64_t total = E * d;
    for (int64_t i = (int64_t)blockIdx.x * blockDim.x + threadIdx.x; i < total; i += (int64_t)gridDim.x * blockDim.x) {
        const int64_t e = i / d, c = i % d;
        const int64_t r = index[e];
        if (r >= 0 && r < N) {
            const float ex = expf(src[i] - mx[r * d + c]);
            out[i] = ex;
            atomicAdd(sum + r * d + c, ex);
        }
    }
}

__global__ void seg_div_kernel(const int64_t* __restrict__ index, int64_t E, int64_t d, int64_t N,
                               const float* __restrict__ sum, float* __restrict__ out) {
    const int64_t total = E * d;
    for (int64_t i = (int64_t)blockIdx.x * blockDim.x + threadIdx.x; i < total; i += (int64_t)gridDim.x * blockDim.x) {
        const int64_t e = i / d, c = i % d;
        const int64_t r = index[e];
        if (r >= 0 && r < N) out[i] = out[i] / sum[r * d + c];
    }
}

inline unsigned grid_for(int64_t total) {
    int64_t g = (total + 255) / 256;
    if (g < 1) g = 1;
    return (unsigned)(g < 16384 ? g : 16384);
}

}

extern "C" {

int jmac_scatter_sum_f32(const float* src, const int64_t* index, int64_t E, int64_t d, int64_t N, float* out,
                         jmac_stream_t stream) {
    if (E < 0 || d <= 0 || N < 0) return JMAC_EINVAL;
    if (E == 0) return JMAC_OK;
    if (!src || !index || !out) return JMAC_EINVAL;
    hipLaunchKernelGGL(scatter_sum_kernel, dim3(grid_for(E * d)), dim3(256), 0, (hipStream_t)stream, src, index, E, d, N, out);
    return (int)hipGetLastError();
}

size_t jmac_scatter_softmax_workspace_bytes(int64_t N, int64_t d) {
    if (N < 0 || d < 0) return 0;
    return 2 * align_up((size_t)N * (size_t)d * 4) + 256;
}

int jmac_scatter_softmax_f32(const float* src, const int64_t* index, int64_t E, int64_t d, int64_t N, float* out, void* ws,
                             size_t ws_bytes, jmac_stream_t stream) {
    if (E < 0 || d <= 0 || N < 0) return JMAC_EINVAL;
    if (E == 0) return JMAC_OK;
    if (!src || !index || !out) return JMAC_EINVAL;
    if (!ws || ws_bytes < jmac_scatter_softmax_workspace_bytes(N, d)) return JMAC_EWORKSPACE;
    hipStream_t st = (hipStream_t)stream;
    float* mx = (float*)ws;
    float* sum = (float*)((char*)ws + align_up((size_t)N * (size_t)d * 4));
    hipLaunchKernelGGL(fill_f32_kernel, dim3(grid_for(N * d)), dim3(256), 0, st, mx, N * d, -INFINITY);
    hipLaunchKernelGGL(fill_f32_kernel, dim3(grid_for(N * d)), dim3(256), 0, st, sum, N * d, 0.f);
    hipLaunchKernelGGL(seg_max_kernel, dim3(grid_for(E * d)), dim3(256), 0, st, src, index, E, d, N, mx);
    hipLaunchKernelGGL(seg_expsum_kernel, dim3(grid_for(E * d)), dim3(256), 0, st, src, index, E, d, N, mx, sum, out);
    hipLaunchKernelGGL(seg_div_kernel, dim3(grid_for(E * d)), dim3(256), 0, st, index, E, d, N, sum, out);
    return (int)hipGetLastError();
}

const char* jmac_strerror(int rc) {
    switch (rc) {
        case JMAC_OK: return "ok";
        case JMAC_EINVAL: return "jmac: invalid argument (null pointer or negative size)";
        case JMAC_EDIM: return "jmac: unsupported dimension (need d % 4 == 0, d <= 512, ld % 4 == 0)";
        case JMAC_EWORKSPACE: return "jmac: workspace missing or too small";
        case JMAC_ERANGE: return "jmac: size exceeds int32 indexing";
        default: break;
    }
    if (rc > 0) return hipGetErrorString((hipError_t)rc);
    return "jmac: unknown error";
}

int jmac_version(void) { return 132; }

}
```

jmac_amd/encoder.py:

```python
from __future__ import annotations

import ctypes as C
from types import SimpleNamespace
from typing import List, Optional, Sequence

import torch
import torch.nn.functional as F

from . import ops
from ._lib import AggFwdJob, GemmTask, check, lib, ptr, require_device, stream
from .graph import RelGraph

ACT_NONE, ACT_LEAKY, ACT_RELU, DACT_LEAKY, DACT_RELU = 0, 1, 2, 3, 4
MAX_TASKS = 24
CAPTURE = None


def gemm_task(A, B, Cout, *, ta=False, tb=False, A2=None, C2=None, act=ACT_NONE, act_src=None, slope=0.0, accumulate=False,
              defer=False):
    for t in (A, B, Cout, A2, C2, act_src):
        if t is not None and (t.dtype != torch.float32 or t.stride(-1) != 1):
            raise TypeError("grouped GEMM operands are fp32 with unit inner stride")
    a_rows = A.shape[0] + (A2.shape[0] if A2 is not None else 0)
    M, K = (A.shape[1], a_rows) if ta else (a_rows, A.shape[1])
# ... 4 lines not shown
    if A2 is not None and (A2.shape[1] != A.shape[1] or A2.stride(0) != A.stride(0)) and A2.shape[0] > 1:
        raise ValueError("A2 must share A's width and leading dimension")
    t = GemmTask()
    t.A, t.A2, t.lda, t.a_split = ptr(A), ptr(A2), A.stride(0), (A.shape[0] if A2 is not None else 0)
    t.transA, t.transB = int(ta), int(tb)
    t.B, t.ldb = ptr(B), B.stride(0)
    t.C, t.C2, t.ldc, t.c_split = ptr(Cout), ptr(C2), Cout.stride(0), (Cout.shape[0] if C2 is not None else 0)
    t.M, t.N, t.K = M, N, K
    t.act_src, t.ld_act_src = ptr(act_src), (act_src.stride(0) if act_src is not None else 0)
    t.act, t.accumulate, t.slope = int(act), int(bool(accumulate)), float(slope)
    t._keep = (A, B, Cout, A2, C2, act_src)
    t._defer = bool(defer)
    t._cost = ((M + 31) // 32) * ((N + 31) // 32) * ((K + 303) // 304)
    return t


def grouped_gemm(tasks: Sequence[GemmTask]) -> None:
    tasks = [t for t in tasks if t is not None]
    for i in range(0, len(tasks), MAX_TASKS):
        chunk = tasks[i:i + MAX_TASKS]
        arr = (GemmTask * len(chunk))(*chunk)
        check(lib().jmac_gemm_grouped_f32(arr, len(chunk), stream()), "jmac_gemm_grouped_f32")


def balance_levels(levels: List[List[GemmTask]]) -> List[List[GemmTask]]:
    levels = [list(lv) for lv in levels]
    while levels and not levels[-1]:
        levels.pop()
    total = sum(t._cost for lv in levels for t in lv)
    if not total or len(levels) < 2:
        return levels
    target = total / len(levels)
    for i in range(len(levels) - 1):
        cost = sum(t._cost for t in levels[i])
        movable = sorted((t for t in levels[i] if t._defer), key=lambda t: -t._cost)
        for t in movable:
            if cost <= target:
                break
            levels[i].remove(t)
            levels[i + 1].append(t)
            cost -= t._cost
    return levels


def run_levels(levels: List[List[GemmTask]], balance: bool = False) -> None:
    for lv in (balance_levels(levels) if balance else levels):
        if lv:
            grouped_gemm(lv)


def _empty(dev, *shape):
    return torch.empty(shape, dtype=torch.float32, device=dev)


PAIR_LAUNCHES = True


def _agg_fwd_pair(specs, graph: RelGraph, out_scale=0.5, compact=False):
    calls = [ops._fwd_call(*ops.pqz_views(PQZ), RR, a, graph, slope, out_scale, RR.shape[0] - 1, 0, compact)
             for PQZ, RR, a, slope in specs]
    jobs = (AggFwdJob * len(calls))(*[AggFwdJob(*args[:-1]) for _, args, _, _ in calls])
    ops._launch(lib().jmac_rel_attn_aggregate_fwd_jobs_f32, (jobs, len(calls), stream()), "rel_attn_fwd_pair")
    return [res for _, _, res, _ in calls]


class RowBlocks:

    def __init__(self, sizes, order=None):
        self.sizes = tuple(int(n) for n in sizes)
        self.nb = len(self.sizes)
        if not 1 <= self.nb <= 16 or min(self.sizes) <= 0:
            raise ValueError("RowBlocks: 1..16 non-empty blocks")
        off = [0]
        for n in self.sizes:
            off.append(off[-1] + n)
        self.offsets = tuple(off)
        self.order = tuple(int(o) for o in (order if order is not None else range(self.nb)))
        if sorted(self.order) != list(range(self.nb)):
            raise ValueError("RowBlocks: order must be a permutation of the blocks")
        self.c_ptr = (C.c_int64 * (self.nb + 1))(*off)
        self.c_order = (C.c_int32 * self.nb)(*self.order)


def _bn_fwd(x, bn, training, y, y2=None, seg=None, norm=None):
    use_batch = bool(training or not bn.track_running_stats)
    if training and bn.track_running_stats:
        if _TRACKERS is not None:
            _TRACKERS.append(bn.num_batches_tracked)
        else:
            bn.num_batches_tracked.add_(seg.nb if seg is not None else 1)
    if norm is not None:
        mean, invstd, norm.inv = ops.bn_tanh_norm_fwd_raw(x, bn.weight, bn.bias, bn.running_mean, bn.running_var, use_batch,
                                                          bn.momentum, bn.eps, y, norm.yn, norm.drop, norm.row_map, norm.y_rows)
        return mean, invstd, use_batch
    mean, invstd = ops.bn_tanh_fwd_raw(x, bn.weight, bn.bias, bn.running_mean, bn.running_var, use_batch, bn.momentum, bn.eps,
                                       y, y2, seg)
    return mean, invstd, use_batch


_bn_bwd = ops.bn_tanh_bwd_raw


def _norm_drop_fwd(x, p_drop, training, y, mask=None, seed=None):
    N, d = x.shape
    inv = _empty(x.device, max(N, 1))
    if not (training and p_drop > 0.0):
        mask = seed = None
    if seed is not None and mask is None:
        check(lib().jmac_row_normalize_dropseed_fwd_f32(ptr(x), x.stride(0), N, d, 1e-12, ptr(seed), float(p_drop), ptr(y),
                                                        y.stride(0), ptr(inv), stream()), "jmac_row_normalize_dropseed_fwd_f32")
        return inv, ("seed", seed, float(p_drop))
    scale = 1.0
    if training and p_drop > 0.0:
        if mask is None:
            mask = torch.empty((N, d), dtype=torch.float32, device=x.device).bernoulli_(1.0 - p_drop)
        scale = 1.0 / (1.0 - p_drop)
    check(lib().jmac_row_normalize_drop_fwd_f32(ptr(x), x.stride(0), N, d, 1e-12, ptr(mask), d, scale, ptr(y), y.stride(0),
                                                ptr(inv), stream()), "jmac_row_normalize_drop_fwd_f32")
    return inv, (("mask", mask, scale) if mask is not None else None)


def _norm_drop_bwd(x, inv, drop, g, gx, accumulate):
    N, d = x.shape
    if drop is not None and drop[0] == "seed":
        check(lib().jmac_row_normalize_dropseed_bwd_f32(ptr(x), x.stride(0), ptr(inv), ptr(drop[1]), drop[2], ptr(g), g.stride(0), N,
                                                        d, 1e-12, ptr(gx), gx.stride(0), 1 if accumulate else 0, stream()),
              "jmac_row_normalize_dropseed_bwd_f32")
        return
    mask, scale = (drop[1], drop[2]) if drop is not None else (None, 1.0)
    check(lib().jmac_row_normalize_drop_bwd_f32(ptr(x), x.stride(0), ptr(inv), ptr(mask), d, scale, ptr(g), g.stride(0), N, d,
                                                1e-12, ptr(gx), gx.stride(0), 1 if accumulate else 0, stream()),
          "jmac_row_normalize_drop_bwd_f32")


FUSE_ROW_PASSES = True


def _fuse_rows_ok(cfg, d) -> bool:
    return bool(FUSE_ROW_PASSES and d <= 512 and cfg.table_dtype == torch.float32 and (cfg.seg is None or cfg.seg.nb == 1))


def _seed_drop(p_drop, training, seed):
    return ("seed", seed, float(p_drop)) if (training and p_drop > 0.0 and seed is not None) else None


def _gather_norm_drop_fwd(x, row_map, p_drop, training, y, seed=None):
    N, d = x.shape
    x = x if x.stride(-1) == 1 else x.contiguous()
    xr, inv = _empty(x.device, N, d), _empty(x.device, max(N, 1))
    drop = _seed_drop(p_drop, training, seed)
    sp, p = ops._seed_args(drop)
    check(lib().jmac_rows_normalize_dropseed_fwd_f32(ptr(x), x.stride(0), ptr(row_map), N, d, 1e-12, sp, p, ptr(xr), xr.stride(0), ptr(y),
                                                     y.stride(0), ptr(inv), stream()), "jmac_rows_normalize_dropseed_fwd_f32")
    return xr, inv, drop


def _norm_drop_bwd_scatter(x, inv, drop, g, add, row_map, dst=None):
    N, d = x.shape
    acc = dst is not None
    if dst is None:
        dst = _empty(x.device, N, d)
    sp, p = ops._seed_args(drop)
    check(lib().jmac_row_normalize_dropseed_bwd_rows_f32(ptr(x), x.stride(0), ptr(inv), sp, p, ptr(g), g.stride(0), ptr(add),
                                                         add.stride(0) if add is not None else 0, ptr(row_map), N, d, 1e-12, ptr(dst),
                                                         dst.stride(0), 1 if acc else 0, stream()),
          "jmac_row_normalize_dropseed_bwd_rows_f32")
    return dst


_TRACKERS = None

INPLACE_GRADS = True
INPLACE_COUNT = 0
# ... 257 lines not shown


class _MlpChain:

    def __init__(self, lay, Ra, L11u, L12u, mlp_slope, W1, W2, loop, wc, d):
        dev, nr = Ra.device, Ra.shape[0]
        self.Ra, self.L11u, self.L12u, self.W1, self.W2, self.loop, self.wc, self.d, self.nr = Ra, L11u, L12u, W1, W2, loop, wc, d, nr
        self.mlp_slope = float(mlp_slope)
        self.relu = lay.rel_activation == "relu"
        self.slope = float(lay.atv_mlp.negative_slope)
        self.M, self.Wp, self.W2g = _empty(dev, nr, L11u.shape[1]), _empty(dev, L12u.shape[0], d), _empty(dev, d, 2 * d)
        self.T, self.RR = _empty(dev, nr + 1, d), _empty(dev, nr + 1, 2 * d)

    def rel_in(self):
        return torch.mm(self.M, self.L12u)

    def fwd_tasks(self):
        act = ACT_RELU if self.relu else ACT_LEAKY
        return [[gemm_task(self.Ra, self.L11u, self.M, act=ACT_LEAKY, slope=self.mlp_slope),
                 gemm_task(self.L12u, self.W1, self.Wp), gemm_task(self.W2, self.wc[:, self.d:], self.W2g)],
                [gemm_task(self.M, self.Wp, self.T[:self.nr], act=act, slope=self.slope),
                 gemm_task(self.loop, self.W1, self.T[self.nr:], act=act, slope=self.slope)],
                [gemm_task(self.T, self.W2g, self.RR)]]

    def bwd_tasks(self, dRR, dwc, dRa, dRa_accumulate):
        dev, d, nr = dRR.device, self.d, self.nr
        dT, dW2g, dM, dWp = _empty(dev, nr + 1, d), _empty(dev, d, 2 * d), _empty(dev, *self.M.shape), _empty(dev, *self.Wp.shape)
        dW1, dW2, dloop = _empty(dev, d, d), _empty(dev, d, d), _empty(dev, 1, d)
        dL11u, dL12u = _empty(dev, *self.L11u.shape), _empty(dev, *self.L12u.shape)
        dact = DACT_RELU if self.relu else DACT_LEAKY
        return [[gemm_task(dRR, self.W2g, dT, tb=True, act=dact, act_src=self.T, slope=self.slope),
                 gemm_task(self.T, dRR, dW2g, ta=True)],
                [gemm_task(dT[:nr], self.Wp, dM, tb=True, act=DACT_LEAKY, act_src=self.M, slope=self.mlp_slope),
                 gemm_task(self.M, dT[:nr], dWp, ta=True),
                 gemm_task(dT[nr:], self.W1, dloop, tb=True),
                 gemm_task(self.loop, dT[nr:], dW1, ta=True),
                 gemm_task(dW2g, self.wc[:, d:], dW2, tb=True, defer=True),
                 gemm_task(self.W2, dW2g, dwc[:, d:], ta=True, accumulate=True, defer=True)],
                [gemm_task(dM, self.L11u, dRa, tb=True, accumulate=dRa_accumulate),
                 gemm_task(self.Ra, dM, dL11u, ta=True),
                 gemm_task(dWp, self.W1, dL12u, tb=True),
                 gemm_task(self.L12u, dWp, dW1, ta=True, accumulate=True)]], (dW1, dW2, dloop), (dL11u, dL12u)


_DEFER = object()


def _layer_fwd(lay, X, wc, RR, a, graph, training, y, y2=None, table_dtype=torch.float32, seg=None, compact=False, rows=None,
               agg=None, norm=None):
    if table_dtype == torch.bfloat16:
        d = wc.shape[0]
        dh = ops.bf16_pad(d)
        PQZ = torch.mm(X.to(torch.bfloat16), ops.pad_table_weight(wc, d, 3).to(torch.bfloat16))
        if dh != d:
            RRp = torch.zeros((RR.shape[0], 2 * dh), dtype=torch.bfloat16, device=RR.device)
            RRp[:, :d] = RR[:, :d]
            RRp[:, dh:dh + d] = RR[:, d:]
            RR = RRp
        else:
            RR = RR.to(torch.bfloat16)
    elif rows is not None:
        d = wc.shape[0]
        PQZ = _empty(X.device, X.shape[0], 3 * d)
        torch.mm(X, wc[:, 2 * d:], out=PQZ[:, 2 * d:])
        for r0, r1 in rows.dst_ranges:
            if r1 > r0:
                torch.mm(X[r0:r1], wc[:, :d], out=PQZ[r0:r1, :d])
        for r0, r1 in rows.src_ranges:
            if r1 > r0:
                torch.mm(X[r0:r1], wc[:, d:2 * d], out=PQZ[r0:r1, d:2 * d])
    else:
        PQZ = torch.mm(X, wc)
    slope = float(lay.atv_mlp.negative_slope)
    if agg is _DEFER:
        return SimpleNamespace(X=X, wc=wc, RR=RR, a=a, PQZ=PQZ, slope=slope)
    if agg is None:
        agg = ops.rel_attn_split_fwd_raw(*ops.pqz_views(PQZ), RR, a, graph, slope, 0.5, RR.shape[0] - 1, 0, compact=compact)
    pre, smax, sden = agg
    mean, invstd, use_batch = _bn_fwd(pre, lay.bn, training, y, y2, seg, norm)
    return SimpleNamespace(X=X, wc=wc, RR=RR, a=a, PQZ=PQZ, pre=pre, smax=smax, sden=sden, y=y, mean=mean, invstd=invstd,
                           use_batch=use_batch, slope=slope, bn_weight=lay.bn.weight, seg=seg, compact=compact, rows=rows)


def _layer_finish(lay, part, agg, training, y, y2=None, seg=None, compact=False, rows=None, norm=None):
    pre, smax, sden = agg
    mean, invstd, use_batch = _bn_fwd(pre, lay.bn, training, y, y2, seg, norm)
    return SimpleNamespace(X=part.X, wc=part.wc, RR=part.RR, a=part.a, PQZ=part.PQZ, pre=pre, smax=smax, sden=sden, y=y, mean=mean,
                           invstd=invstd, use_batch=use_batch, slope=part.slope, bn_weight=lay.bn.weight, seg=seg, compact=compact,
                           rows=rows)


def _layer_bwd(st, graph, gy, gy2, dX, dX_accumulate, adj=None):
    if adj is not None:
        gpre, gbw = ops.bn_tanh_bwd_normadj_raw(st.pre, st.y, adj.inv, adj.drop, adj.g, gy2, adj.row_map, st.bn_weight, st.mean,
                                                st.invstd, st.use_batch)
    else:
        gpre, gbw = _bn_bwd(st.pre, st.y, gy, gy2, st.bn_weight, st.mean, st.invstd, st.use_batch, st.seg)
    dPQZ = _empty(st.PQZ.device, *st.PQZ.shape)
    _, _, dRR, da = ops.rel_attn_split_bwd_raw(*ops.pqz_views(st.PQZ), st.RR, st.a, graph, st.slope, 0.5, st.RR.shape[0] - 1, 0,
                                               st.pre, st.smax, st.sden, gpre, compact=st.compact, dPQZ=dPQZ)
    rows = getattr(st, "rows", None)
    if dX is not None and rows is not None:
        d = st.wc.shape[0]
        if dX_accumulate:
            dX.addmm_(dPQZ[:, 2 * d:], st.wc[:, 2 * d:].t())
        else:
            torch.mm(dPQZ[:, 2 * d:], st.wc[:, 2 * d:].t(), out=dX)
        for r0, r1 in rows.dst_ranges:
            if r1 > r0:
                dX[r0:r1].addmm_(dPQZ[r0:r1, :d], st.wc[:, :d].t())
        for r0, r1 in rows.src_ranges:
            if r1 > r0:
                dX[r0:r1].addmm_(dPQZ[r0:r1, d:2 * d], st.wc[:, d:2 * d].t())
    elif dX is not None:
        if dX_accumulate:
            dX.addmm_(dPQZ, st.wc.t())
        else:
            torch.mm(dPQZ, st.wc.t(), out=dX)
    dwc = torch.mm(st.X.t(), dPQZ)
    return dRR, dwc, da, gbw


def _layer_grads(chain_grads, dwatt_dgcn, da, gbw, d):
    dW1, dW2, dloop = chain_grads
    d_watt, d_gcn = dwatt_dgcn
    return [dW1, dW2, dloop, d_watt, da.view(d, 1), d_gcn, gbw[d:], gbw[:d]]


def _layer_ok(l, d) -> bool:
    slope = float(l.atv_mlp.negative_slope)
    return (l.comp_op == "sub" and l.layer_act is torch.tanh and l.bn.momentum is not None and l.bn.affine
            and l.in_channels == d and l.out_channels == d and 0.0 <= slope <= 1.0
            and getattr(l, "fused", True) and getattr(l, "bwd_mode", ops.BWD_MODE_DETERMINISTIC) == ops.BWD_MODE_DETERMINISTIC
            and not l._forward_hooks and not l._forward_pre_hooks)


def supported(model, info_dim: Optional[int]) -> bool:
    a = model.args
    d = model.entity_dim
    lays = (model.conv1_alignment, model.conv2_alignment, model.conv1_completion)
    return (getattr(a, "num_gcn_layer", 2) == 2 and d % 4 == 0 and (info_dim is None or info_dim % 4 == 0)
            and _tables_ok(getattr(model, "table_dtype", torch.float32))
            and 0.0 <= float(model.atv_mlp.negative_slope) <= 1.0 and float(model.completion_dropout.p) < 1.0
            and len({l.chunk for l in lays}) == 1
            and all(_layer_ok(l, d) and _tables_ok(l.table_dtype) for l in lays))


def _tables_ok(dtype) -> bool:
    return dtype == torch.float32 or (dtype == torch.bfloat16 and not torch.is_grad_enabled())


class _LayerNode(torch.autograd.Function):

    @staticmethod
    def forward(ctx, cfg, X, R, *pl):
        require_device(X, R)
        (lay,) = cfg.layers
        N, d = X.shape
        t = SimpleNamespace()
        (t.wc,) = _wcat_pack([pl[3]], [pl[5]], d)
        t.rc = _RelCompact(cfg.graph, R.shape[0])
        (Ru,) = t.rc.gather([R])
        t.ch = _Chain(lay, Ru, pl[0], pl[1], pl[2], t.wc, d)
        w2g, tt, rr = t.ch.fwd_tasks()
        run_levels([[w2g, tt], [rr]])
        y = _empty(X.device, N, d)
        t.st = _layer_fwd(lay, X, t.wc, t.ch.RR, pl[4].reshape(-1), cfg.graph, cfg.training, y, seg=cfg.seg, compact=t.rc.on)
        t.st.y = None
        if CAPTURE is not None:
# ... 144 lines not shown
        slot.busy, slot.lease = True, slot.lease + 1
        return _Cat0Lease(slot, slot.buf, True)
    buf = _empty(dev, N, d + di)
    buf[:, d:].copy_(info)
    if slots is not None and slot is None and len(slots) < CAT0_MAX_SLOTS and not torch.cuda.is_current_stream_capturing():
        slot = slots[key] = _Cat0Slot()
        slot.buf, slot.info, slot.busy, slot.lease = buf, info, True, 1
        return _Cat0Lease(slot, buf, True)
    return _Cat0Lease(_Cat0Slot(), buf, False)


class _EncoderName(torch.autograd.Function):

    @staticmethod
    def forward(ctx, cfg, *tensors):
        global _TRACKERS
        _TRACKERS = []
        try:
            out = _EncoderName._forward(ctx, cfg, *tensors)
            done = {id(c) for c in ctx.t.bumped}
            _bump_trackers([c for c in _TRACKERS if id(c) not in done])
            if cfg.seg is not None and cfg.seg.nb > 1 and ctx.t.bumped:
                torch._foreach_add_(ctx.t.bumped, cfg.seg.nb - 1)
            return out
        finally:
            _TRACKERS = None

    @staticmethod
    def _forward(ctx, cfg, E, Rc, Ra, info, NL, U11, U21, Wall, L11, L12, L11u, L12u, *lp):
        require_device(E, Rc, Ra, info)
        ctx.set_materialize_grads(False)
        la, lc, l2 = cfg.layers
        pa, pc, p2 = lp[0:8], lp[8:16], lp[16:24]
        graph, training, p_drop, mslope = cfg.graph, cfg.training, cfg.p_drop, cfg.mlp_slope
        dev = E.device
        N, d = E.shape
        di = info.shape[1]
        t = SimpleNamespace()
        t.ro = ro = _row_order(cfg, graph, N)
        t.fuse = fuse = _fuse_rows_ok(cfg, d)
        E_n, info_n = E, info
        if ro is not None:
            graph = ro.graph
            if not fuse:
                (E_n,) = _gather_rows([E], ro.old_of_new)
            info_n = ro.info_rows(info)
        t.w = _empty(dev, d + di, d)
        u11 = U11.contiguous()
        t.bumped = [lay.bn.num_batches_tracked for lay in (la, lc, l2) if training and lay.bn.track_running_stats]
        seeds = None
        if training and p_drop > 0.0:
            state = _drop_seed_state(cfg.cache, dev)
            seeds = (state, torch.empty(2, dtype=torch.int64, device=dev)) if state is not None else None
        t.wc = _wcat_pack([p[3] for p in (pa, pc, p2)], [p[5] for p in (pa, pc, p2)], d, copy=(u11[:d], t.w[:d]),
                          counters=t.bumped, seed=seeds)
        (Ra_u,), fc, mc = _completion_rel_fwd(t, graph, lc, pc, t.wc[1], Rc, L11, L12, mslope, d, also=[Ra])
        t.cha = _Chain(la, Ra_u, pa[0], pa[1], pa[2], t.wc[0], d)
        t.ch2 = _MlpChain(l2, Ra_u, L11u, L12u, mslope, p2[0], p2[1], p2[2], t.wc[2], d)
        fa, f2 = t.cha.fwd_tasks(), t.ch2.fwd_tasks()
        run_levels([[fa[0], fa[1], fc[0], fc[1], *f2[0], mc[0], gemm_task(NL, U11[d:], t.w[d:])],
                    [fa[2], fc[2], *f2[1], mc[1]],
                    f2[2]])
        t.cat0_lease = _cat0_take(cfg.cache, info_n, N, d, dev, persistent=cfg.info_persistent)
        t.cat0, t.cat1, t.catA = t.cat0_lease.buf, _empty(dev, N, 2 * d), _empty(dev, N, 3 * d)
        seeds = (seeds[1] if seeds is not None
                 else (torch.empty(2, dtype=torch.int64, device=dev).random_() if training and p_drop > 0.0 else None))
        sd = (lambda i: seeds[i:i + 1]) if seeds is not None else (lambda i: None)
        if fuse and ro is not None:
            E_n, t.inv0, t.drop0 = _gather_norm_drop_fwd(E, ro.old_of_new, p_drop, training, t.cat0[:, :d], seed=sd(0))
        else:
            t.inv0, t.drop0 = _norm_drop_fwd(E_n, p_drop, training, t.cat0[:, :d], seed=sd(0))
        align0 = t.catA[:, :d]
        torch.mm(t.cat0, t.w, out=align0)
        a_att = [p[4].reshape(-1) for p in (pa, pc, p2)]
        seg = cfg.seg
        c1 = _empty(dev, N, d)
        c1_out = _empty(dev, N, d) if (fuse and ro is not None) else None
        norm = (SimpleNamespace(yn=t.cat1[:, :d], drop=_seed_drop(p_drop, training, sd(1)), y_rows=c1_out,
                                row_map=ro.old_of_new if ro is not None else None, inv=None) if fuse else None)
        if PAIR_LAUNCHES and cfg.table_dtype == torch.float32:
            pa_ = _layer_fwd(la, align0, t.wc[0], t.cha.RR, a_att[0], graph, training, None, rows=ro, agg=_DEFER)
            pc_ = _layer_fwd(lc, E_n, t.wc[1], t.chc.RR, a_att[1], graph, training, None, rows=ro, agg=_DEFER)
            ra, rc_ = _agg_fwd_pair([(pa_.PQZ, pa_.RR, pa_.a, pa_.slope), (pc_.PQZ, pc_.RR, pc_.a, pc_.slope)], graph, compact=t.rc.on)
            t.sa = _layer_finish(la, pa_, ra, training, t.catA[:, d:2 * d], t.cat1[:, d:], seg=seg, compact=t.rc.on, rows=ro)
            t.sc = _layer_finish(lc, pc_, rc_, training, c1, seg=seg, compact=t.rc.on, rows=ro, norm=norm)
        else:
            t.sa = _layer_fwd(la, align0, t.wc[0], t.cha.RR, a_att[0], graph, training, t.catA[:, d:2 * d], t.cat1[:, d:],
                              table_dtype=cfg.table_dtype, seg=seg, compact=t.rc.on, rows=ro)
            t.sc = _layer_fwd(lc, E_n, t.wc[1], t.chc.RR, a_att[1], graph, training, c1, table_dtype=cfg.table_dtype, seg=seg,
                              compact=t.rc.on, rows=ro, norm=norm)
        if norm is not None:
            t.inv1, t.drop1 = norm.inv, norm.drop
        else:
            t.inv1, t.drop1 = _norm_drop_fwd(c1, p_drop, training, t.cat1[:, :d], seed=sd(1))
        t.a_in = torch.mm(t.cat1, U21)
        t.s2 = _layer_fwd(l2, t.a_in, t.wc[2], t.ch2.RR, a_att[2], graph, training, t.catA[:, 2 * d:],
                          table_dtype=cfg.table_dtype, seg=seg, compact=t.rc.on, rows=ro)
        align_out = torch.mm(t.catA, Wall)
        if ro is not None:
            t.E_n, t.c1_n = E_n, c1
            if c1_out is not None:
                (align_out,), c1 = _gather_rows([align_out], ro.new_of_old), c1_out
            else:
                align_out, c1 = _gather_rows([align_out, c1], ro.new_of_old)
        if CAPTURE is not None:
            back = (lambda x: x[ro.new_of_old]) if ro is not None else (lambda x: x.clone())
            rel_a_in = torch.mm(F.leaky_relu(torch.mm(Ra.detach(), L11u.detach()), mslope), L12u.detach())
            _capture_layer("conv1_alignment", back(align0), Ra.detach(), t.sa, t.cha, t.rc, ro)
            _capture_layer("conv2_alignment", back(t.a_in), rel_a_in, t.s2, t.ch2, t.rc, ro)
            CAPTURE["rel_used"] = graph.rel_used if t.rc.on else None
            CAPTURE["rel_linear11.act"], CAPTURE["rel_linear11_uni.act"] = t.mlc.M, t.ch2.M
        rel_c1 = _completion_outputs(t, E, Rc, ro)
        ctx.t, ctx.cfg, ctx.dims = t, cfg, (N, d, di)
        ctx.save_for_backward(E, Rc, Ra, NL, U11, U21, Wall, L11, L12, L11u, L12u, c1)
        return align_out, c1, rel_c1, E, Rc

    @staticmethod
    def backward(ctx, g_align, g_c1, g_relc1, g_E0, g_Rc0):
        t, cfg = ctx.t, ctx.cfg
        N, d, di = ctx.dims
        E, Rc, Ra, NL, U11, U21, Wall, L11, L12, L11u, L12u, c1 = ctx.saved_tensors
        ro = t.ro
        E_x, c1_y = (t.E_n, t.c1_n) if ro is not None else (E, c1)
        graph = ro.graph if ro is not None else cfg.graph
        dev = E.device
        have_align = g_align is not None
        have_c = have_align or g_c1 is not None
        fuse = t.fuse and not torch.is_grad_enabled()
        adj_c = fuse and have_align
        if ro is not None and have_c:
            gin = [g for g in (g_align, None if adj_c else g_c1) if g is not None]
            gout = _gather_rows(gin, ro.old_of_new)
            if g_align is not None:
                g_align = gout[0]
            if g_c1 is not None and not adj_c:
                g_c1 = gout[-1]
        dE = dRa = e_adj = None
        dRc = g_Rc0
        dWall = dU21 = dU11 = dNL = gL11 = gL12 = gL11u = gL12u = None
        ga = gc = g2 = [None] * 8
        levels: List[List[GemmTask]] = [[] for _ in range(5)]
        if have_align:
            g_align = g_align.contiguous()
            dcatA = torch.mm(g_align, Wall.t())
            dWall = torch.mm(t.catA.t(), g_align)
            d_ain = _empty(dev, N, d)
            dRR2, dwc2, da2, gbw2 = _layer_bwd(t.s2, graph, dcatA[:, 2 * d:], None, d_ain, False)
            dcat1 = torch.mm(d_ain, U21.t())
            dU21 = torch.mm(t.cat1.t(), d_ain)
        if have_c:
            gy, gy2, adj = None, None, None
            if have_align:
                gy2 = g_c1.contiguous() if g_c1 is not None else None
                if adj_c:
                    adj = SimpleNamespace(inv=t.inv1, drop=t.drop1, g=dcat1[:, :d], row_map=ro.old_of_new if ro is not None else None)
                else:
                    gy = _empty(dev, N, d)
                    _norm_drop_bwd(c1_y, t.inv1, t.drop1, dcat1[:, :d], gy, False)
            else:
                gy = g_c1.contiguous()
            dE, g_E0, (dRRc, dwcc, dac, gbwc) = _completion_layer_bwd(t, c1_y, graph, gy, gy2, g_E0, take=ro is None, adj=adj)
        if have_align:
            d_align0 = dcatA[:, :d]
            dRRa, dwca, daa, gbwa = _layer_bwd(t.sa, graph, dcatA[:, d:2 * d], dcat1[:, d:], d_align0, True)
            d_comp0 = torch.mm(d_align0, t.w[:d].t())
            t.cat0_lease.check()
            dw = torch.mm(t.cat0.t(), d_align0)
            t.cat0_lease.release()
# ... 106 lines not shown
```

jmac_amd/ops.py:

```python
from __future__ import annotations

import ctypes as C
from typing import Optional, Tuple

import torch

from ._lib import check, lib, ptr, require_device, stream, testing_lib, workspace
from .graph import RelGraph

BWD_MODE_ATOMIC = 0
BWD_MODE_DETERMINISTIC = 1

PROFILE = None


def _ev():
    e = torch.cuda.Event(enable_timing=True)
    e.record()
    return e


def _launch(fn, args, name: str) -> None:
    if PROFILE is None:
        check(fn(*args), fn.__name__)
        return
    ev0 = _ev()
    check(fn(*args), fn.__name__)
    PROFILE.append((name, ev0, _ev()))


def _f32c(t: torch.Tensor) -> torch.Tensor:
    if t.dtype != torch.float32:
        raise TypeError("jmac_amd ops compute in fp32 (got %s)" % t.dtype)
    return t


def _table(t: torch.Tensor) -> torch.Tensor:
    if t.dtype not in (torch.float32, torch.bfloat16):
        raise TypeError("jmac_amd tables are fp32 or bf16 (got %s)" % t.dtype)
    return t


def bf16_pad(d: int) -> int:
    return 304 if d == 300 else d


def pad_table_weight(w: torch.Tensor, d: int, parts: int) -> torch.Tensor:
    dh = bf16_pad(d)
    if dh == d:
        return w
    out = w.new_zeros((w.shape[0], parts * dh))
    for p_ in range(parts):
        out[:, p_ * dh:p_ * dh + d] = w[:, p_ * d:(p_ + 1) * d]
    return out


def pad_table(t: torch.Tensor, d: int, parts: int) -> torch.Tensor:
    return pad_table_weight(t, d, parts)


def pqz_views(PQZ: torch.Tensor):
    dh = PQZ.shape[1] // 3
    return PQZ[:, :dh], PQZ[:, dh:]


class _RelAttnAggregate(torch.autograd.Function):

    @staticmethod
    def forward(ctx, PQZ, RR, a, graph: RelGraph, slope: float, loop_rel: int, out_scale: float, bwd_mode: int):
        require_device(PQZ, RR, a)
        PQZ, RR, a = _table(PQZ).contiguous(), _table(RR).contiguous(), _f32c(a).contiguous()
        out, seg_max, seg_den = rel_attn_split_fwd_raw(*pqz_views(PQZ), RR, a, graph, slope, out_scale, loop_rel, 0)
        if PQZ.dtype == torch.bfloat16:
            ctx.mark_non_differentiable(out)
            return out
        ctx.save_for_backward(PQZ, RR, a, out, seg_max, seg_den)
        ctx.graph, ctx.slope, ctx.loop_rel, ctx.out_scale, ctx.bwd_mode = graph, slope, loop_rel, out_scale, bwd_mode
        return out

    @staticmethod
    def backward(ctx, G):
        PQZ, RR, a, out, seg_max, seg_den = ctx.saved_tensors
        dPQZ = torch.empty_like(PQZ)
        _, _, dRR, da = rel_attn_split_bwd_raw(*pqz_views(PQZ), RR, a, ctx.graph, ctx.slope, ctx.out_scale, ctx.loop_rel, 0, out,
                                               seg_max, seg_den, G, mode=int(ctx.bwd_mode), dPQZ=dPQZ)
        return dPQZ, dRR, da, None, None, None, None, None


def rel_attn_aggregate(PQZ: torch.Tensor, RR: torch.Tensor, a: torch.Tensor, graph: RelGraph, slope: float,
                       loop_rel: int = -1, out_scale: float = 1.0,
# ... 162 lines not shown
def rel_attn_aggregate_split(P, QZ, RR, a, graph: RelGraph, slope: float, out_scale: float = 1.0, loop_rel: int = -1,
                             self_off: int = 0) -> torch.Tensor:
    return _RelAttnAggregateSplit.apply(P, QZ, RR, a, graph, float(slope), float(out_scale), int(loop_rel), int(self_off))


def bn_tanh_fwd_raw(x, weight, bias, running_mean, running_var, training: bool, momentum: float, eps: float, y, y2=None,
                    seg=None):
    L = lib()
    N, d = x.shape
    dev = x.device
    ldy2 = y2.stride(0) if y2 is not None else 0
    if training and seg is not None and seg.nb > 1:
        if seg.offsets[-1] != N:
            raise ValueError("RowBlocks cover %d rows, the layer has %d" % (seg.offsets[-1], N))
        mean = torch.empty((seg.nb, d), dtype=torch.float32, device=dev)
        invstd = torch.empty((seg.nb, d), dtype=torch.float32, device=dev)
        ws_bytes = int(L.jmac_bn_tanh_seg_workspace_bytes(seg.nb, d))
        ws = workspace(ws_bytes, dev)
        check(L.jmac_bn_tanh_seg_fwd2_f32(ptr(x), x.stride(0), d, seg.nb, seg.c_ptr, seg.c_order, ptr(weight), ptr(bias),
                                          ptr(running_mean), ptr(running_var), float(momentum), float(eps), ptr(y), y.stride(0),
                                          ptr(y2), ldy2, ptr(mean), ptr(invstd), ptr(ws), ws_bytes, stream()),
              "jmac_bn_tanh_seg_fwd2_f32")
        return mean, invstd
    mean = torch.empty(d, dtype=torch.float32, device=dev)
    invstd = torch.empty(d, dtype=torch.float32, device=dev)
    ws_bytes = int(L.jmac_bn_tanh_workspace_bytes(N, d))
    ws = workspace(ws_bytes, dev)
    check(L.jmac_bn_tanh_fwd2_f32(ptr(x), x.stride(0), N, d, ptr(weight), ptr(bias), ptr(running_mean), ptr(running_var),
                                  1 if training else 0, float(momentum), float(eps), ptr(y), y.stride(0), ptr(y2), ldy2, ptr(mean),
                                  ptr(invstd), ptr(ws), ws_bytes, stream()), "jmac_bn_tanh_fwd2_f32")
    return mean, invstd


def bn_tanh_bwd_raw(x, y, gy, gy2, weight, mean, invstd, training: bool, seg=None):
    L = lib()
    N, d = x.shape
    dev = x.device
    gx = torch.empty((N, d), dtype=torch.float32, device=dev)
    gbw = torch.empty(2 * d, dtype=torch.float32, device=dev)
    ldgy2 = gy2.stride(0) if gy2 is not None else 0
    if mean.dim() == 2:
        ws_bytes = int(L.jmac_bn_tanh_seg_workspace_bytes(seg.nb, d))
        ws = workspace(ws_bytes, dev)
        check(L.jmac_bn_tanh_seg_bwd2_f32(ptr(x), x.stride(0), ptr(y), y.stride(0), ptr(gy), gy.stride(0), ptr(gy2), ldgy2, d,
                                          seg.nb, seg.c_ptr, ptr(weight), ptr(mean), ptr(invstd), ptr(gx), d,
                                          gbw.data_ptr() + d * 4, ptr(gbw), ptr(ws), ws_bytes, stream()),
              "jmac_bn_tanh_seg_bwd2_f32")
        return gx, gbw
    ws_bytes = int(L.jmac_bn_tanh_workspace_bytes(N, d))
    ws = workspace(ws_bytes, dev)
    check(L.jmac_bn_tanh_bwd2_f32(ptr(x), x.stride(0), ptr(y), y.stride(0), ptr(gy), gy.stride(0), ptr(gy2), ldgy2, N, d,
                                  ptr(weight), ptr(mean), ptr(invstd), 1 if training else 0, ptr(gx), d, gbw.data_ptr() + d * 4,
                                  ptr(gbw), ptr(ws), ws_bytes, stream()), "jmac_bn_tanh_bwd2_f32")
    return gx, gbw


def _seed_args(drop):
    if drop is None:
        return None, 0.0
    if drop[0] != "seed":
        raise ValueError("the fused row passes draw from a device seed (mask-form dropout keeps the separate launches)")
    return ptr(drop[1]), float(drop[2])


def bn_tanh_norm_fwd_raw(x, weight, bias, running_mean, running_var, training: bool, momentum: float, eps: float, y, yn, drop,
                         row_map=None, y_rows=None):
    L = lib()
    N, d = x.shape
    dev = x.device
    mean = torch.empty(d, dtype=torch.float32, device=dev)
    invstd = torch.empty(d, dtype=torch.float32, device=dev)
    inv = torch.empty(max(N, 1), dtype=torch.float32, device=dev)
    seed, p_drop = _seed_args(drop)
    ws_bytes = int(L.jmac_bn_tanh_workspace_bytes(N, d))
    ws = workspace(ws_bytes, dev)
    check(L.jmac_bn_tanh_normalize_dropseed_fwd_f32(ptr(x), x.stride(0), N, d, ptr(weight), ptr(bias), ptr(running_mean),
                                                    ptr(running_var), 1 if training else 0, float(momentum), float(eps), ptr(y),
                                                    y.stride(0), ptr(row_map), ptr(y_rows), y_rows.stride(0) if y_rows is not None else 0,
                                                    1e-12, seed, p_drop, ptr(yn), yn.stride(0), ptr(inv), ptr(mean), ptr(invstd),
                                                    ptr(ws), ws_bytes, stream()), "jmac_bn_tanh_normalize_dropseed_fwd_f32")
    return mean, invstd, inv


def bn_tanh_bwd_normadj_raw(x, y, inv, drop, g, gy2, row_map, weight, mean, invstd, training: bool):
    L = lib()
    N, d = x.shape
    dev = x.device
    gx = torch.empty((N, d), dtype=torch.float32, device=dev)
    gbw = torch.empty(2 * d, dtype=torch.float32, device=dev)
    seed, p_drop = _seed_args(drop)
    ws_bytes = int(L.jmac_bn_tanh_workspace_bytes(N, d))
    ws = workspace(ws_bytes, dev)
    check(L.jmac_bn_tanh_bwd_normadj_f32(ptr(x), x.stride(0), ptr(y), y.stride(0), ptr(inv), ptr(g), g.stride(0), 1e-12, seed, p_drop,
                                         ptr(gy2), gy2.stride(0) if gy2 is not None else 0, ptr(row_map), N, d, ptr(weight), ptr(mean),
                                         ptr(invstd), 1 if training else 0, ptr(gx), d, gbw.data_ptr() + d * 4, ptr(gbw), ptr(ws),
                                         ws_bytes, stream()), "jmac_bn_tanh_bwd_normadj_f32")
    return gx, gbw


class _BnTanh(torch.autograd.Function):

    @staticmethod
    def forward(ctx, x, weight, bias, running_mean, running_var, training: bool, momentum: float, eps: float):
        require_device(x, weight, bias)
        x = _f32c(x).contiguous()
        y = torch.empty_like(x)
        save_mean, save_invstd = bn_tanh_fwd_raw(x, weight, bias, running_mean, running_var, training, momentum, eps, y)
        ctx.save_for_backward(x, y, weight, save_mean, save_invstd)
        ctx.training = training
        return y

    @staticmethod
    def backward(ctx, gy):
        x, y, weight, save_mean, save_invstd = ctx.saved_tensors
        d = x.shape[1]
        gx, gbw = bn_tanh_bwd_raw(x, y, _f32c(gy).contiguous(), None, weight, save_mean, save_invstd, ctx.training)
        return gx, gbw[d:], gbw[:d], None, None, None, None, None


def bn_tanh(x, weight, bias, running_mean, running_var, training: bool, momentum: float = 0.1, eps: float = 1e-5):
    if x.shape[1] % 4 != 0:
        raise ValueError("bn_tanh needs d % 4 == 0 (pad on the host)")
    return _BnTanh.apply(x, weight, bias, running_mean, running_var, bool(training), float(momentum), float(eps))


def _gemm(A, ta, B, tb, M, N, K):
    C_ = torch.empty((M, N), dtype=torch.float32, device=A.device)
    check(lib().jmac_gemm_f32(ptr(A), A.stride(0), 1 if ta else 0, ptr(B), B.stride(0), 1 if tb else 0, M, N, K, ptr(C_), N,
                              stream()), "jmac_gemm_f32")
    return C_


def _rowmajor(t: torch.Tensor) -> torch.Tensor:
    return t if (t.dim() == 2 and t.stride(1) == 1) else t.contiguous()


class _SmallMM(torch.autograd.Function):

    @staticmethod
    def forward(ctx, A, B):
        require_device(A, B)
        A, B = _rowmajor(_f32c(A)), _rowmajor(_f32c(B))
        if A.shape[1] != B.shape[0]:
            raise ValueError("small_mm: %s @ %s" % (tuple(A.shape), tuple(B.shape)))
        ctx.save_for_backward(A, B)
        return _gemm(A, False, B, False, A.shape[0], B.shape[1], A.shape[1])

    @staticmethod
    def backward(ctx, G):
        A, B = ctx.saved_tensors
        G = _rowmajor(_f32c(G))
        M, K = A.shape
        N = B.shape[1]
        dA = _gemm(G, False, B, True, M, K, N) if ctx.needs_input_grad[0] else None
        dB = _gemm(A, True, G, False, K, N, M) if ctx.needs_input_grad[1] else None
        return dA, dB


def _gemm_any(A: torch.Tensor, B: torch.Tensor) -> torch.Tensor:
    def operand(t):
        if t.stride(1) == 1:
            return t, False
        if t.stride(0) == 1:
            return t.t(), True
        return t.contiguous(), False
    (a, ta), (b, tb) = operand(A), operand(B)
# ... 71 lines not shown
```

jmac_amd/optim.py:

```python
from __future__ import annotations

import torch

from ._lib import AdamTask, check, lib, ptr, stream


class Adam(torch.optim.Optimizer):
    _decoupled = False

    def __init__(self, params, lr=1e-3, betas=(0.9, 0.999), eps=1e-8, weight_decay=0.0, amsgrad=False, *, maximize=False):
        if amsgrad:
            raise NotImplementedError("jmac_amd.optim.Adam: amsgrad is not offered (the reference trains without it: train.py:406-407)")
        if isinstance(lr, torch.Tensor):
            raise TypeError("jmac_amd.optim.Adam: lr is a host number (it is a kernel argument)")
        if not 0.0 <= lr or not 0.0 <= eps or not 0.0 <= weight_decay or not 0.0 <= betas[0] < 1.0 or not 0.0 <= betas[1] < 1.0:
            raise ValueError("jmac_amd.optim.Adam: invalid hyper-parameter (lr=%r betas=%r eps=%r weight_decay=%r)"
                             % (lr, betas, eps, weight_decay))
        super().__init__(params, dict(lr=lr, betas=tuple(betas), eps=eps, weight_decay=weight_decay, amsgrad=False, maximize=maximize))
        self._managed = {}
        self._tables = {}
        self._keep = []

    @staticmethod
    def _aux(v, betas, dev):
        return torch.tensor([betas[0] ** v, betas[1] ** v, 0.0], dtype=torch.float64).to(dev)

    def _counters(self, ps, dev, betas):
        capturing = torch.cuda.is_current_stream_capturing()
        adopt = {}
        for p in ps:
            st = self.state[p]
            c = st.get("step")
            if c is not None and id(c) in self._managed and self._managed[id(c)][0] is c:
                continue
            if capturing:
                raise RuntimeError("jmac_amd.optim.Adam: the first step of a parameter (or the first after load_state_dict) reads "
                                   "its step count on the host: run one step outside the hipGraph capture first")
            v = 0.0 if c is None else float(c)
            cn = adopt.get(v)
            if cn is None:
                cn = adopt[v] = torch.full((), v, dtype=torch.float32, device=dev)
                self._managed[id(cn)] = [cn, set(), self._aux(v, betas, dev), betas]
            self._managed[id(cn)][1].add(id(p))
            st["step"] = cn
        groups = {}
        for p in ps:
            c = self.state[p]["step"]
            groups.setdefault(id(c), (c, []))[1].append(p)
        out = []
        for cid, (c, plist) in groups.items():
            members = self._managed[cid][1]
            if len(plist) != len(members):
                if capturing:
                    raise RuntimeError("jmac_amd.optim.Adam: the set of parameters with gradients changed inside a hipGraph capture")
                c2 = c.clone()
                mine = set(id(p) for p in plist)
                self._managed[id(c2)] = [c2, mine, self._managed[cid][2].clone(), self._managed[cid][3]]
                members -= mine
                for p in plist:
                    self.state[p]["step"] = c2
                c = c2
            rec = self._managed[id(c)]
            if rec[3] != betas:
                if capturing:
                    raise RuntimeError("jmac_amd.optim.Adam: betas changed inside a hipGraph capture")
                rec[2], rec[3] = self._aux(float(c), betas, dev), betas
            out.append((c, plist, rec[2]))
        return out

    def _group_step(self, group):
        ps = [p for p in group["params"] if p.grad is not None]
        if not ps:
            return
        dev = ps[0].device
        for p in ps:
            if p.device != dev or not p.is_cuda or p.dtype != torch.float32 or p.grad.dtype != torch.float32 or p.grad.is_sparse:
                raise TypeError("jmac_amd.optim.Adam: fp32 parameters with dense fp32 gradients on one HIP device (there is no CPU path)")
            if not p.is_contiguous():
                raise ValueError("jmac_amd.optim.Adam: parameters must be contiguous")
            st = self.state[p]
            if "exp_avg" not in st:
                st["exp_avg"] = torch.zeros_like(p, memory_format=torch.contiguous_format)
                st["exp_avg_sq"] = torch.zeros_like(p, memory_format=torch.contiguous_format)
            for k in ("exp_avg", "exp_avg_sq"):
                if st[k].dtype != torch.float32 or not st[k].is_contiguous() or st[k].device != dev:
                    st[k] = st[k].to(device=dev, dtype=torch.float32).contiguous()
        b1, b2 = (float(b) for b in group["betas"])
        for counter, plist, aux in self._counters(ps, dev, (b1, b2)):
            tasks = []
            for p in plist:
                st = self.state[p]
                g = p.grad if p.grad.is_contiguous() else p.grad.contiguous()
                tasks.append((p, g, st["exp_avg"], st["exp_avg_sq"]))
            key = tuple((t[0].data_ptr(), t[1].data_ptr(), t[2].data_ptr(), t[3].data_ptr(), t[0].numel()) for t in tasks)
            cached = self._tables.get(id(counter))
            if cached is None or cached[0] != key:
                table = (AdamTask * len(tasks))()
                for i, (p, g, m, v) in enumerate(tasks):
                    table[i].p, table[i].g, table[i].m, table[i].v, table[i].n, table[i].vec4 = ptr(p), ptr(g), ptr(m), ptr(v), p.numel(), 0
                cached = self._tables[id(counter)] = (key, table)
            check(lib().jmac_adam_step_f32(cached[1], len(tasks), ptr(counter), ptr(aux), float(group["lr"]), b1, b2,
                                           float(group["eps"]), float(group["weight_decay"]), 1 if self._decoupled else 0,
                                           1 if group["maximize"] else 0, stream()), "jmac_adam_step_f32")
            self._keep.append(tasks)

    def state_dict(self):
        sd = super().state_dict()
        host = {}

        def to_host(t):
            key = (t.data_ptr(), t.device)
            if key not in host:
                host[key] = t.detach().to("cpu", copy=True)
            return host[key].clone()
        sd["state"] = {k: {**v, "step": to_host(v["step"])} if "step" in v else dict(v) for k, v in sd["state"].items()}
        return sd

    @torch.no_grad()
    def step(self, closure=None):
        loss = None
        if closure is not None:
            with torch.enable_grad():
                loss = closure()
        self._keep = []
        for group in self.param_groups:
            self._group_step(group)
        return loss


class AdamW(Adam):
    _decoupled = True

    def __init__(self, params, lr=1e-3, betas=(0.9, 0.999), eps=1e-8, weight_decay=1e-2, amsgrad=False, *, maximize=False):
        super().__init__(params, lr=lr, betas=betas, eps=eps, weight_decay=weight_decay, amsgrad=amsgrad, maximize=maximize)
```

Before: 31.28 million.

## Batch paired BatchNorm-tanh forward statistics into shared multi-job kernel launches

Adds a job-table entry point that runs the column-statistics and reduce-finalize kernels for two BatchNorm-tanh layers in single launches, partitioning blocks between jobs by index. The model's paired alignment and context layers now call this batched path instead of two separate forward calls. This is meant to cut launch count and let the two small reductions share the GPU. The Adam optimizer also gains per-chunk auxiliary slots sized by a new library query, which changes its aux buffer layout.

```diff
diff --git a/include/jmac_hip.h b/include/jmac_hip.h
--- a/include/jmac_hip.h
+++ b/include/jmac_hip.h
@@ -202,6 +202,15 @@
                                              int64_t ldadd, const int64_t* row_map, int64_t N, int64_t d, float eps,
                                              float* dst, int64_t lddst, int32_t accumulate, jmac_stream_t stream);
 
+typedef struct {
+    const float *x; int64_t ldx, N, d; const float *weight, *bias; float *running_mean, *running_var; float momentum, eps;
+    float *y; int64_t ldy; float *y2; int64_t ldy2;
+    int32_t norm; const int64_t *row_map; float *y_rows; int64_t ldyr; float norm_eps; const int64_t *seed; float p_drop;
+    float *yn; int64_t ldyn; float *inv;
+    float *save_mean, *save_invstd; void *ws; size_t ws_bytes;
+} jmac_bn_fwd_job_t;
+int jmac_bn_tanh_fwd_jobs_f32(const jmac_bn_fwd_job_t* jobs, int32_t n_jobs, jmac_stream_t stream);
+
 int jmac_l1_score_f32(const float* er, int64_t lder, const float* table, int64_t ldt, int64_t B,
                       int64_t N, int64_t d, float* out, int64_t ldout, int32_t accumulate,
                       jmac_stream_t stream);
@@ -360,6 +369,7 @@
     int64_t n;
     int32_t vec4;
 } jmac_adam_task_t;
+int64_t jmac_adam_slots(const jmac_adam_task_t* tasks, int32_t n_tasks);
 int jmac_adam_step_f32(const jmac_adam_task_t* tasks, int32_t n_tasks, float* step, double* aux, double lr, double beta1,
                        double beta2, double eps, double weight_decay, int32_t decoupled, int32_t maximize, jmac_stream_t stream);
 
diff --git a/jmac_amd/_lib.py b/jmac_amd/_lib.py
--- a/jmac_amd/_lib.py
+++ b/jmac_amd/_lib.py
@@ -37,6 +37,13 @@
     _fields_ = [("P", vp), ("ldp", i64), ("QZ", vp), ("ldqz", i64), ("RR", vp), ("ldrr", i64), ("a_att", vp), ("col", vp), ("etype", vp),
                 ("by_dst", C.POINTER(View)), ("N", i64), ("d", i64), ("slope", f32), ("loop_rel", i32), ("self_off", i64),
                 ("out_scale", f32), ("out", vp), ("ldo", i64), ("seg_max", vp), ("seg_den", vp), ("ws", vp), ("ws_bytes", sz)]
+
+
+class BnFwdJob(C.Structure):
+    _fields_ = [("x", vp), ("ldx", i64), ("N", i64), ("d", i64), ("weight", vp), ("bias", vp), ("running_mean", vp),
+                ("running_var", vp), ("momentum", f32), ("eps", f32), ("y", vp), ("ldy", i64), ("y2", vp), ("ldy2", i64),
+                ("norm", i32), ("row_map", vp), ("y_rows", vp), ("ldyr", i64), ("norm_eps", f32), ("seed", vp), ("p_drop", f32),
+                ("yn", vp), ("ldyn", i64), ("inv", vp), ("save_mean", vp), ("save_invstd", vp), ("ws", vp), ("ws_bytes", sz)]
 
 
 class AdamTask(C.Structure):
@@ -97,12 +104,14 @@
     "jmac_rows_normalize_dropseed_fwd_f32": (C.c_int, [vp, i64, vp, i64, i64, f32, vp, f32, vp, i64, vp, i64, vp, vp]),
     "jmac_bn_tanh_normalize_dropseed_fwd_f32": (C.c_int, [vp, i64, i64, i64, vp, vp, vp, vp, i32, f32, f32, vp, i64, vp, vp, i64,
                                                           f32, vp, f32, vp, i64, vp, vp, vp, vp, sz, vp]),
+    "jmac_bn_tanh_fwd_jobs_f32": (C.c_int, [C.POINTER(BnFwdJob), i32, vp]),
     "jmac_bn_tanh_bwd_normadj_f32": (C.c_int, [vp, i64, vp, i64, vp, vp, i64, f32, vp, f32, vp, i64, vp, i64, i64, vp, vp, vp,
                                                i32, vp, i64, vp, vp, vp, sz, vp]),
     "jmac_row_normalize_dropseed_bwd_rows_f32": (C.c_int, [vp, i64, vp, vp, f32, vp, i64, vp, i64, vp, i64, i64, f32, vp, i64,
                                                            i32, vp]),
     "jmac_gemm_grouped_f32": (C.c_int, [C.POINTER(GemmTask), i32, vp]),
     "jmac_wcat_pack_seed_f32": (C.c_int, [C.POINTER(vp), C.POINTER(vp), C.POINTER(vp), i32, i64, vp, vp, i64, C.POINTER(vp), i32, vp, vp, vp]),
+    "jmac_adam_slots": (i64, [C.POINTER(AdamTask), i32]),
     "jmac_adam_step_f32": (C.c_int, [C.POINTER(AdamTask), i32, vp, vp, C.c_double, C.c_double, C.c_double, C.c_double, C.c_double, i32, i32,
                                      vp]),
     "jmac_wcat_unpack_f32": (C.c_int, [C.POINTER(vp), C.POINTER(vp), C.POINTER(vp), i32, i64, vp, vp, i64, vp]),
diff --git a/jmac_amd/csrc/norm.hip b/jmac_amd/csrc/norm.hip
--- a/jmac_amd/csrc/norm.hip
+++ b/jmac_amd/csrc/norm.hip
@@ -9,8 +9,8 @@
 constexpr int kBlock = 256;
 constexpr int kStatBlocks = 512;
 
-__global__ __launch_bounds__(kBlock) void col_stats_partial_kernel(const float* __restrict__ x, int64_t ldx, int64_t N,
-                                                                   int D4, float* __restrict__ partial) {
+__device__ __forceinline__ void col_stats_partial_body(const float* __restrict__ x, int64_t ldx, int64_t N, int D4,
+                                                       float* __restrict__ partial, const int bid, const int nblk) {
     extern __shared__ __attribute__((aligned(16))) char smem[];
     float4* red = reinterpret_cast<float4*>(smem);
     const int rpb = kBlock / D4 > 0 ? kBlock / D4 : 1;
@@ -22,7 +22,7 @@
         float4 s1 = f4zero(), s2 = f4zero();
         if (active) {
             const float4 K = ld4(x + c4 * 4);
-            for (int64_t r = (int64_t)blockIdx.x * rpb + rsub; r < N; r += (int64_t)gridDim.x * rpb) {
+            for (int64_t r = (int64_t)bid * rpb + rsub; r < N; r += (int64_t)nblk * rpb) {
                 float4 v = ld4(x + r * ldx + c4 * 4);
                 v.x -= K.x; v.y -= K.y; v.z -= K.z; v.w -= K.w;
                 s1.x += v.x; s1.y += v.y; s1.z += v.z; s1.w += v.w;
@@ -31,8 +31,8 @@
         }
         if (D4 >= kBlock) {
             if (active) {
-                st4(partial + ((int64_t)blockIdx.x * 2 + 0) * D4 * 4 + c4 * 4, s1);
-                st4(partial + ((int64_t)blockIdx.x * 2 + 1) * D4 * 4 + c4 * 4, s2);
+                st4(partial + ((int64_t)bid * 2 + 0) * D4 * 4 + c4 * 4, s1);
+                st4(partial + ((int64_t)bid * 2 + 1) * D4 * 4 + c4 * 4, s2);
             }
         } else {
             if (active) {
@@ -47,12 +47,30 @@
                     a1.x += b1.x; a1.y += b1.y; a1.z += b1.z; a1.w += b1.w;
                     a2.x += b2.x; a2.y += b2.y; a2.z += b2.z; a2.w += b2.w;
                 }
-                st4(partial + ((int64_t)blockIdx.x * 2 + 0) * D4 * 4 + tid * 4, a1);
-                st4(partial + ((int64_t)blockIdx.x * 2 + 1) * D4 * 4 + tid * 4, a2);
+                st4(partial + ((int64_t)bid * 2 + 0) * D4 * 4 + tid * 4, a1);
+                st4(partial + ((int64_t)bid * 2 + 1) * D4 * 4 + tid * 4, a2);
             }
             break;
         }
     }
+}
+
+__global__ __launch_bounds__(kBlock) void col_stats_partial_kernel(const float* __restrict__ x, int64_t ldx, int64_t N,
+                                                                   int D4, float* __restrict__ partial) {
+    col_stats_partial_body(x, ldx, N, D4, partial, (int)blockIdx.x, (int)gridDim.x);
+}
+
+struct StatArgs {
+    const float* x;
+    int64_t ldx, N;
+    int D4;
+    float* partial;
+};
+__global__ __launch_bounds__(kBlock) void col_stats_partial_jobs_kernel(StatArgs a0, StatArgs a1, int g0) {
+    if ((int)blockIdx.x < g0)
+        col_stats_partial_body(a0.x, a0.ldx, a0.N, a0.D4, a0.partial, (int)blockIdx.x, g0);
+    else
+        col_stats_partial_body(a1.x, a1.ldx, a1.N, a1.D4, a1.partial, (int)blockIdx.x - g0, (int)gridDim.x - g0);
 }
 
 __global__ void bn_finalize_kernel(const float* __restrict__ sums, const float* __restrict__ x, int64_t N,
@@ -78,14 +96,22 @@
 }
 
 constexpr int RF_COLS = 16, RF_LANES = 1024 / RF_COLS;
-__global__ __launch_bounds__(1024) void bn_reduce_finalize_kernel(const float* __restrict__ partial, int nparts,
-                                                                  const float* __restrict__ x, int64_t N, int d, float eps,
-                                                                  float momentum, float* __restrict__ running_mean,
-                                                                  float* __restrict__ running_var, float* __restrict__ save_mean,
-                                                                  float* __restrict__ save_invstd) {
-    __shared__ float red1[RF_LANES][RF_COLS], red2[RF_LANES][RF_COLS];
+struct FinArgs {
+    const float* partial;
+    int nparts;
+    const float* x;
+    int64_t N;
+    int d;
+    float eps, momentum;
+    float *running_mean, *running_var, *save_mean, *save_invstd;
+};
+__device__ __forceinline__ void bn_reduce_finalize_body(const float* __restrict__ partial, int nparts, const float* __restrict__ x,
+                                                        int64_t N, int d, float eps, float momentum,
+                                                        float* __restrict__ running_mean, float* __restrict__ running_var,
+                                                        float* __restrict__ save_mean, float* __restrict__ save_invstd, const int bid,
+                                                        float (&red1)[RF_LANES][RF_COLS], float (&red2)[RF_LANES][RF_COLS]) {
     const int cl = threadIdx.x % RF_COLS, rl = threadIdx.x / RF_COLS;
-    const int c = blockIdx.x * RF_COLS + cl;
+    const int c = bid * RF_COLS + cl;
     float a1 = 0.f, a2 = 0.f, b1 = 0.f, b2 = 0.f;
     if (c < d) {
         int p = rl;
@@ -123,6 +149,26 @@
             running_var[c] = (1.f - momentum) * running_var[c] + momentum * unbiased;
         }
     }
+}
+
+__global__ __launch_bounds__(1024) void bn_reduce_finalize_kernel(const float* __restrict__ partial, int nparts,
+                                                                  const float* __restrict__ x, int64_t N, int d, float eps,
+                                                                  float momentum, float* __restrict__ running_mean,
+                                                                  float* __restrict__ running_var, float* __restrict__ save_mean,
+                                                                  float* __restrict__ save_invstd) {
+    __shared__ float red1[RF_LANES][RF_COLS], red2[RF_LANES][RF_COLS];
+    bn_reduce_finalize_body(partial, nparts, x, N, d, eps, momentum, running_mean, running_var, save_mean, save_invstd,
+                            (int)blockIdx.x, red1, red2);
+}
+
+__global__ __launch_bounds__(1024) void bn_reduce_finalize_jobs_kernel(FinArgs a0, FinArgs a1, int g0) {
+    __shared__ float red1[RF_LANES][RF_COLS], red2[RF_LANES][RF_COLS];
+    if ((int)blockIdx.x < g0)
+        bn_reduce_finalize_body(a0.partial, a0.nparts, a0.x, a0.N, a0.d, a0.eps, a0.momentum, a0.running_mean, a0.running_var,
+                                a0.save_mean, a0.save_invstd, (int)blockIdx.x, red1, red2);
+    else
+        bn_reduce_finalize_body(a1.partial, a1.nparts, a1.x, a1.N, a1.d, a1.eps, a1.momentum, a1.running_mean, a1.running_var,
+                                a1.save_mean, a1.save_invstd, (int)blockIdx.x - g0, red1, red2);
 }
 
 __global__ void moments_finalize_kernel(const float* __restrict__ sums, const float* __restrict__ x, int64_t N, int d,
@@ -1229,40 +1275,115 @@
 constexpr int kDropRows = 4;
 constexpr int64_t kDropRowsMinN = 2048;
 
-}
-
-extern "C" {
-
-size_t jmac_bn_tanh_workspace_bytes(int64_t N, int64_t d) {
-    (void)N;
-    return align_up((size_t)(kStatBlocks + 1) * 2 * (d > 0 ? d : 0) * 4) + 256;
-}
-
-int jmac_bn_tanh_fwd2_f32(const float* x, int64_t ldx, int64_t N, int64_t d, const float* weight, const float* bias,
-                          float* running_mean, float* running_var, int32_t training, float momentum, float eps, float* y,
-                          int64_t ldy, float* y2, int64_t ldy2, float* save_mean, float* save_invstd, void* ws, size_t ws_bytes,
-                          jmac_stream_t stream) {
+enum BnPhase { kBnAll, kBnCheck, kBnApply };
+
+int seeded_src(const int64_t* seed, float p_drop, DropSrc& ds) {
+    if (!seed || !(p_drop >= 0.f) || !(p_drop < 1.f)) return JMAC_EINVAL;
+    const double keep = 1.0 - (double)p_drop, t = keep * 4294967296.0;
+    ds = DropSrc{nullptr, 0, seed, t >= 4294967295.0 ? 0xFFFFFFFFu : (uint32_t)t, (float)(1.0 / keep)};
+    return JMAC_OK;
+}
+
+int fused_src(const int64_t* seed, float p_drop, DropSrc& ds) {
+    if (seed) return seeded_src(seed, p_drop, ds);
+    ds = DropSrc{nullptr, 0, nullptr, 0u, 1.f};
+    return JMAC_OK;
+}
+bool aligned16(std::initializer_list<const void*> ps) {
+    uintptr_t a = 0;
+    for (const void* p : ps) a |= (uintptr_t)p;
+    return (a & 15) == 0;
+}
+unsigned rows_grid(int64_t N, int R) {
+    int64_t rb = ((N + R - 1) / R + kBlock / 64 - 1) / (kBlock / 64);
+    return (unsigned)(rb > 8192 ? 8192 : rb);
+}
+#define JMAC_LAUNCH_SEEDED(kernel, R, grid, st, ...)                                                                      \
+    do {                                                                                                                  \
+        if (ds.seed) hipLaunchKernelGGL((kernel<true, R>), dim3(grid), dim3(kBlock), 0, st, __VA_ARGS__);                 \
+        else hipLaunchKernelGGL((kernel<false, R>), dim3(grid), dim3(kBlock), 0, st, __VA_ARGS__);                        \
+    } while (0)
+#define JMAC_LAUNCH_ADJ(kernel, R, grid, st, ...)                                                                         \
+    do {                                                                                                                  \
+        const bool rowform = N >= kDropRowsMinN;                                                                          \
+        if (ds.seed && rowform) hipLaunchKernelGGL((kernel<true, true, R>), dim3(grid), dim3(kBlock), 0, st, __VA_ARGS__); \
+        else if (ds.seed) hipLaunchKernelGGL((kernel<true, false, R>), dim3(grid), dim3(kBlock), 0, st, __VA_ARGS__);     \
+        else if (rowform) hipLaunchKernelGGL((kernel<false, true, R>), dim3(grid), dim3(kBlock), 0, st, __VA_ARGS__);     \
+        else hipLaunchKernelGGL((kernel<false, false, R>), dim3(grid), dim3(kBlock), 0, st, __VA_ARGS__);                 \
+    } while (0)
+
+void bn_stats(const float* x, int64_t ldx, int64_t N, int64_t d, float* running_mean, float* running_var, int32_t training,
+                     float momentum, float eps, float* save_mean, float* save_invstd, void* ws, hipStream_t st) {
+    if (training) {
+        const int D4 = (int)(d / 4);
+        float* partial = (float*)ws;
+        const unsigned g = stat_grid(N, D4);
+        hipLaunchKernelGGL(col_stats_partial_kernel, dim3(g), dim3(kBlock), stat_smem(D4), st, x, ldx, N, D4, partial);
+        hipLaunchKernelGGL(bn_reduce_finalize_kernel, dim3((unsigned)((d + RF_COLS - 1) / RF_COLS)), dim3(1024), 0, st, partial,
+                           (int)g, x, N, (int)d, eps, momentum, running_mean, running_var, save_mean, save_invstd);
+    } else {
+        hipLaunchKernelGGL(bn_eval_stats_kernel, dim3((unsigned)((d + 255) / 256)), dim3(256), 0, st, running_mean, running_var,
+                           (int)d, eps, save_mean, save_invstd);
+    }
+}
+
+int bn_tanh_fwd2(const float* x, int64_t ldx, int64_t N, int64_t d, const float* weight, const float* bias,
+                        float* running_mean, float* running_var, int32_t training, float momentum, float eps, float* y,
+                        int64_t ldy, float* y2, int64_t ldy2, float* save_mean, float* save_invstd, void* ws, size_t ws_bytes,
+                        jmac_stream_t stream, BnPhase phase) {
     if (N < 0 || !weight || !bias || !save_mean || !save_invstd) return JMAC_EINVAL;
     if (d <= 0 || d % 4 || ldx % 4 || ldy % 4 || (y2 && ldy2 % 4)) return JMAC_EDIM;
     if (N == 0) return JMAC_OK;
     if (!x || !y) return JMAC_EINVAL;
     hipStream_t st = (hipStream_t)stream;
     const int D4 = (int)(d / 4);
-    if (training) {
-        if (!ws || ws_bytes < jmac_bn_tanh_workspace_bytes(N, d)) return JMAC_EWORKSPACE;
-        float* partial = (float*)ws;
-        const unsigned g = stat_grid(N, D4);
-        hipLaunchKernelGGL(col_stats_partial_kernel, dim3(g), dim3(kBlock), stat_smem(D4), st, x, ldx, N, D4, partial);
-        hipLaunchKernelGGL(bn_reduce_finalize_kernel, dim3((unsigned)((d + RF_COLS - 1) / RF_COLS)), dim3(1024), 0, st, partial,
-                           (int)g, x, N, (int)d, eps, momentum, running_mean, running_var, save_mean, save_invstd);
-    } else {
-        if (!running_mean || !running_var) return JMAC_EINVAL;
-        hipLaunchKernelGGL(bn_eval_stats_kernel, dim3((unsigned)((d + 255) / 256)), dim3(256), 0, st, running_mean, running_var,
-                           (int)d, eps, save_mean, save_invstd);
-    }
+    if (training && (!ws || ws_bytes < jmac_bn_tanh_workspace_bytes(N, d))) return JMAC_EWORKSPACE;
+    if (!training && (!running_mean || !running_var)) return JMAC_EINVAL;
+    if (phase == kBnCheck) return JMAC_OK;
+    if (phase == kBnAll) bn_stats(x, ldx, N, d, running_mean, running_var, training, momentum, eps, save_mean, save_invstd, ws, st);
     hipLaunchKernelGGL(bn_tanh_apply_kernel, dim3(stream_grid(N * D4)), dim3(kBlock), 0, st, x, ldx, N, D4, weight, bias,
                        save_mean, save_invstd, y, ldy, y2, ldy2);
     return (int)hipGetLastError();
+}
+
+int bn_tanh_normalize_dropseed_fwd(const float* x, int64_t ldx, int64_t N, int64_t d, const float* weight, const float* bias,
+                                          float* running_mean, float* running_var, int32_t training, float momentum, float eps,
+                                          float* y, int64_t ldy, const int64_t* row_map, float* y_rows, int64_t ldyr, float norm_eps,
+                                          const int64_t* seed, float p_drop, float* yn, int64_t ldyn, float* inv, float* save_mean,
+                                          float* save_invstd, void* ws, size_t ws_bytes, jmac_stream_t stream, BnPhase phase) {
+    DropSrc ds;
+    if (int rc = fused_src(seed, p_drop, ds)) return rc;
+    if (N < 0 || !weight || !bias || !save_mean || !save_invstd || (row_map == nullptr) != (y_rows == nullptr)) return JMAC_EINVAL;
+    if (d <= 0 || d > 512 || d % 4 || ldx % 4 || ldy % 4 || ldyn % 4 || (y_rows && ldyr % 4)) return JMAC_EDIM;
+    if (N == 0) return JMAC_OK;
+    if (!x || !y || !yn || !inv) return JMAC_EINVAL;
+    if (!aligned16({x, y, y_rows, yn, weight, bias, save_mean, save_invstd})) return JMAC_EDIM;
+    hipStream_t st = (hipStream_t)stream;
+    const int D4 = (int)(d / 4);
+    if (training && (!ws || ws_bytes < jmac_bn_tanh_workspace_bytes(N, d))) return JMAC_EWORKSPACE;
+    if (!training && (!running_mean || !running_var)) return JMAC_EINVAL;
+    if (phase == kBnCheck) return JMAC_OK;
+    if (phase == kBnAll) bn_stats(x, ldx, N, d, running_mean, running_var, training, momentum, eps, save_mean, save_invstd, ws, st);
+    JMAC_LAUNCH_SEEDED(bn_tanh_normalize_drop_fwd_kernel, kFuseRows, rows_grid(N, kFuseRows), st, x, ldx, N, D4, weight, bias,
+                       (const float*)save_mean, (const float*)save_invstd, y, ldy, row_map, y_rows, ldyr, norm_eps, ds, yn, ldyn, inv);
+    return (int)hipGetLastError();
+}
+
+}
+
+extern "C" {
+
+size_t jmac_bn_tanh_workspace_bytes(int64_t N, int64_t d) {
+    (void)N;
+    return align_up((size_t)(kStatBlocks + 1) * 2 * (d > 0 ? d : 0) * 4) + 256;
+}
+
+int jmac_bn_tanh_fwd2_f32(const float* x, int64_t ldx, int64_t N, int64_t d, const float* weight, const float* bias,
+                          float* running_mean, float* running_var, int32_t training, float momentum, float eps, float* y,
+                          int64_t ldy, float* y2, int64_t ldy2, float* save_mean, float* save_invstd, void* ws, size_t ws_bytes,
+                          jmac_stream_t stream) {
+    return bn_tanh_fwd2(x, ldx, N, d, weight, bias, running_mean, running_var, training, momentum, eps, y, ldy, y2, ldy2, save_mean,
+                        save_invstd, ws, ws_bytes, stream, kBnAll);
 }
 
 int jmac_bn_tanh_bwd2_f32(const float* x, int64_t ldx, const float* y, int64_t ldy, const float* gy, int64_t ldgy,
@@ -1377,13 +1498,6 @@
     return (int)hipGetLastError();
 }
 
-static int seeded_src(const int64_t* seed, float p_drop, DropSrc& ds) {
-    if (!seed || !(p_drop >= 0.f) || !(p_drop < 1.f)) return JMAC_EINVAL;
-    const double keep = 1.0 - (double)p_drop, t = keep * 4294967296.0;
-    ds = DropSrc{nullptr, 0, seed, t >= 4294967295.0 ? 0xFFFFFFFFu : (uint32_t)t, (float)(1.0 / keep)};
-    return JMAC_OK;
-}
-
 int jmac_row_normalize_drop_fwd_f32(const float* x, int64_t ldx, int64_t N, int64_t d, float eps, const float* mask, int64_t ldm,
                                     float scale, float* y, int64_t ldy, float* inv, jmac_stream_t stream) {
     return drop_fwd(x, ldx, N, d, eps, DropSrc{mask, ldm, nullptr, 0u, scale}, false, y, ldy, inv, stream);
@@ -1409,34 +1523,6 @@
     if (int rc = seeded_src(seed, p_drop, ds)) return rc;
     return drop_bwd(x, ldx, inv, ds, true, g, ldg, N, d, eps, gx, ldgx, accumulate, stream);
 }
-
-static int fused_src(const int64_t* seed, float p_drop, DropSrc& ds) {
-    if (seed) return seeded_src(seed, p_drop, ds);
-    ds = DropSrc{nullptr, 0, nullptr, 0u, 1.f};
-    return JMAC_OK;
-}
-static bool aligned16(std::initializer_list<const void*> ps) {
-    uintptr_t a = 0;
-    for (const void* p : ps) a |= (uintptr_t)p;
-    return (a & 15) == 0;
-}
-static unsigned rows_grid(int64_t N, int R) {
-    int64_t rb = ((N + R - 1) / R + kBlock / 64 - 1) / (kBlock / 64);
-    return (unsigned)(rb > 8192 ? 8192 : rb);
-}
-#define JMAC_LAUNCH_SEEDED(kernel, R, grid, st, ...)                                                                      \
-    do {                                                                                                                  \
-        if (ds.seed) hipLaunchKernelGGL((kernel<true, R>), dim3(grid), dim3(kBlock), 0, st, __VA_ARGS__);                 \
-        else hipLaunchKernelGGL((kernel<false, R>), dim3(grid), dim3(kBlock), 0, st, __VA_ARGS__);                        \
-    } while (0)
-#define JMAC_LAUNCH_ADJ(kernel, R, grid, st, ...)                                                                         \
-    do {                                                                                                                  \
-        const bool rowform = N >= kDropRowsMinN;                                                                          \
-        if (ds.seed && rowform) hipLaunchKernelGGL((kernel<true, true, R>), dim3(grid), dim3(kBlock), 0, st, __VA_ARGS__); \
-        else if (ds.seed) hipLaunchKernelGGL((kernel<true, false, R>), dim3(grid), dim3(kBlock), 0, st, __VA_ARGS__);     \
-        else if (rowform) hipLaunchKernelGGL((kernel<false, true, R>), dim3(grid), dim3(kBlock), 0, st, __VA_ARGS__);     \
-        else hipLaunchKernelGGL((kernel<false, false, R>), dim3(grid), dim3(kBlock), 0, st, __VA_ARGS__);                 \
-    } while (0)
 
 int jmac_rows_normalize_dropseed_fwd_f32(const float* x, int64_t ldx, const int64_t* row_map, int64_t N, int64_t d, float eps,
                                          const int64_t* seed, float p_drop, float* x_rows, int64_t ldxr, float* y, int64_t ldy,
@@ -1458,30 +1544,54 @@
                                             float* y, int64_t ldy, const int64_t* row_map, float* y_rows, int64_t ldyr, float norm_eps,
                                             const int64_t* seed, float p_drop, float* yn, int64_t ldyn, float* inv, float* save_mean,
                                             float* save_invstd, void* ws, size_t ws_bytes, jmac_stream_t stream) {
-    DropSrc ds;
-    if (int rc = fused_src(seed, p_drop, ds)) return rc;
-    if (N < 0 || !weight || !bias || !save_mean || !save_invstd || (row_map == nullptr) != (y_rows == nullptr)) return JMAC_EINVAL;
-    if (d <= 0 || d > 512 || d % 4 || ldx % 4 || ldy % 4 || ldyn % 4 || (y_rows && ldyr % 4)) return JMAC_EDIM;
-    if (N == 0) return JMAC_OK;
-    if (!x || !y || !yn || !inv) return JMAC_EINVAL;
-    if (!aligned16({x, y, y_rows, yn, weight, bias, save_mean, save_invstd})) return JMAC_EDIM;
+    return bn_tanh_normalize_dropseed_fwd(x, ldx, N, d, weight, bias, running_mean, running_var, training, momentum, eps, y, ldy,
+                                          row_map, y_rows, ldyr, norm_eps, seed, p_drop, yn, ldyn, inv, save_mean, save_invstd, ws,
+                                          ws_bytes, stream, kBnAll);
+}
+
+int jmac_bn_tanh_fwd_jobs_f32(const jmac_bn_fwd_job_t* jobs, int32_t n_jobs, jmac_stream_t stream) {
+    if (!jobs || n_jobs < 1 || n_jobs > 2) return JMAC_EINVAL;
+    auto run = [&](const jmac_bn_fwd_job_t& q, BnPhase ph) {
+        if (q.norm)
+            return bn_tanh_normalize_dropseed_fwd(q.x, q.ldx, q.N, q.d, q.weight, q.bias, q.running_mean, q.running_var, 1, q.momentum,
+                                                  q.eps, q.y, q.ldy, q.row_map, q.y_rows, q.ldyr, q.norm_eps, q.seed, q.p_drop, q.yn,
+                                                  q.ldyn, q.inv, q.save_mean, q.save_invstd, q.ws, q.ws_bytes, stream, ph);
+        return bn_tanh_fwd2(q.x, q.ldx, q.N, q.d, q.weight, q.bias, q.running_mean, q.running_var, 1, q.momentum, q.eps, q.y, q.ldy,
+                            q.y2, q.ldy2, q.save_mean, q.save_invstd, q.ws, q.ws_bytes, stream, ph);
+    };
+    for (int k = 0; k < n_jobs; ++k)
+        if (int rc = run(jobs[k], kBnCheck)) return rc;
+    const bool pair = n_jobs == 2 && jobs[0].N > 0 && jobs[1].N > 0;
+    if (!pair) {
+        for (int k = 0; k < n_jobs; ++k)
+            if (int rc = run(jobs[k], kBnAll)) return rc;
+        return JMAC_OK;
+    }
+    {
+        const char *w0 = (const char*)jobs[0].ws, *w1 = (const char*)jobs[1].ws;
+        if (w0 < w1 + jmac_bn_tanh_workspace_bytes(jobs[1].N, jobs[1].d) && w1 < w0 + jmac_bn_tanh_workspace_bytes(jobs[0].N, jobs[0].d))
+            return JMAC_EINVAL;
+    }
     hipStream_t st = (hipStream_t)stream;
-    const int D4 = (int)(d / 4);
-    if (training) {
-        if (!ws || ws_bytes < jmac_bn_tanh_workspace_bytes(N, d)) return JMAC_EWORKSPACE;
-        float* partial = (float*)ws;
-        const unsigned g = stat_grid(N, D4);
-        hipLaunchKernelGGL(col_stats_partial_kernel, dim3(g), dim3(kBlock), stat_smem(D4), st, x, ldx, N, D4, partial);
-        hipLaunchKernelGGL(bn_reduce_finalize_kernel, dim3((unsigned)((d + RF_COLS - 1) / RF_COLS)), dim3(1024), 0, st, partial,
-                           (int)g, x, N, (int)d, eps, momentum, running_mean, running_var, save_mean, save_invstd);
-    } else {
-        if (!running_mean || !running_var) return JMAC_EINVAL;
-        hipLaunchKernelGGL(bn_eval_stats_kernel, dim3((unsigned)((d + 255) / 256)), dim3(256), 0, st, running_mean, running_var,
-                           (int)d, eps, save_mean, save_invstd);
-    }
-    JMAC_LAUNCH_SEEDED(bn_tanh_normalize_drop_fwd_kernel, kFuseRows, rows_grid(N, kFuseRows), st, x, ldx, N, D4, weight, bias,
-                       (const float*)save_mean, (const float*)save_invstd, y, ldy, row_map, y_rows, ldyr, norm_eps, ds, yn, ldyn, inv);
-    return (int)hipGetLastError();
+    StatArgs s[2];
+    FinArgs f[2];
+    unsigned g[2], fg[2];
+    size_t smem = 0;
+    for (int k = 0; k < 2; ++k) {
+        const jmac_bn_fwd_job_t& q = jobs[k];
+        const int D4 = (int)(q.d / 4);
+        g[k] = stat_grid(q.N, D4);
+        fg[k] = (unsigned)((q.d + RF_COLS - 1) / RF_COLS);
+        smem = stat_smem(D4) > smem ? stat_smem(D4) : smem;
+        s[k] = StatArgs{q.x, q.ldx, q.N, D4, (float*)q.ws};
+        f[k] = FinArgs{(const float*)q.ws, (int)g[k], q.x, q.N, (int)q.d, q.eps, q.momentum, q.running_mean, q.running_var, q.save_mean,
+                       q.save_invstd};
+    }
+    hipLaunchKernelGGL(col_stats_partial_jobs_kernel, dim3(g[0] + g[1]), dim3(kBlock), smem, st, s[0], s[1], (int)g[0]);
+    hipLaunchKernelGGL(bn_reduce_finalize_jobs_kernel, dim3(fg[0] + fg[1]), dim3(1024), 0, st, f[0], f[1], (int)fg[0]);
+    for (int k = 0; k < 2; ++k)
+        if (int rc = run(jobs[k], kBnApply)) return rc;
+    return JMAC_OK;
 }
 
 int jmac_bn_tanh_bwd_normadj_f32(const float* x, int64_t ldx, const float* y, int64_t ldy, const float* inv, const float* g,
diff --git a/jmac_amd/csrc/optim.hip b/jmac_amd/csrc/optim.hip
--- a/jmac_amd/csrc/optim.hip
+++ b/jmac_amd/csrc/optim.hip
@@ -12,6 +12,7 @@
     int decoupled, maximize, advance;
     float* step;
     double* aux;
+    double* pow;
 };
 
 struct AdamConst {
@@ -61,8 +62,10 @@
         }
     }
     AdamConst c;
+    double pw1 = 1.0, pw2 = 1.0;
+    if (a.n_chunks > 0) { pw1 = a.pow[2 * (int64_t)ch]; pw2 = a.pow[2 * (int64_t)ch + 1]; }
     {
-        const double bc1 = 1.0 - a.aux[0] * a.beta1, bc2 = 1.0 - a.aux[1] * a.beta2;
+        const double bc1 = 1.0 - pw1 * a.beta1, bc2 = 1.0 - pw2 * a.beta2;
         c.one_minus_b1 = (float)(1.0 - a.beta1);
         c.b2 = (float)a.beta2;
         c.one_minus_b2 = (float)(1.0 - a.beta2);
@@ -97,37 +100,48 @@
             T.p[base + i] = pp; T.m[base + i] = mm; T.v[base + i] = vv;
         }
     }
-    if (a.advance) {
+    if (a.n_chunks > 0) {
         __syncthreads();
         if (threadIdx.x == 0) {
-            unsigned int* ticket = reinterpret_cast<unsigned int*>(a.aux + 2);
-            const unsigned int done = __hip_atomic_fetch_add(ticket, 1u, __ATOMIC_RELAXED, __HIP_MEMORY_SCOPE_AGENT);
-            if (done == gridDim.x - 1) {
-                a.step[0] = a.step[0] + 1.f;
-                a.aux[0] = a.aux[0] * a.beta1;
-                a.aux[1] = a.aux[1] * a.beta2;
-                __hip_atomic_store(ticket, 0u, __ATOMIC_RELAXED, __HIP_MEMORY_SCOPE_AGENT);
-            }
+            a.pow[2 * (int64_t)ch] = pw1 * a.beta1;
+            a.pow[2 * (int64_t)ch + 1] = pw2 * a.beta2;
         }
+    }
+    if (a.advance && ch == 0 && threadIdx.x == 0) {
+        a.step[0] = a.step[0] + 1.f;
+        a.aux[0] = a.aux[0] * a.beta1;
+        a.aux[1] = a.aux[1] * a.beta2;
     }
 }
 
-template <int V>
+constexpr int kAdamV = 1;
+constexpr int kAdamChunk = kAdamBlock * 4 * kAdamV;
+
+inline bool bad_task(const jmac_adam_task_t& t) { return t.n < 0 || (t.n > 0 && (!t.p || !t.g || !t.m || !t.v)); }
+
+int64_t adam_chunks(const jmac_adam_task_t* tasks, int32_t n_tasks) {
+    int64_t chunks = 0;
+    for (int32_t i = 0; i < n_tasks; ++i) {
+        if (tasks[i].n < 0) return -1;
+        chunks += (tasks[i].n + kAdamChunk - 1) / kAdamChunk;
+        if (chunks >= INT32_MAX) return -1;
+    }
+    return chunks;
+}
+
 int launch_adam(const jmac_adam_task_t* tasks, int32_t n_tasks, float* step, double* aux, double lr, double beta1, double beta2,
                 double eps, double weight_decay, int32_t decoupled, int32_t maximize, hipStream_t st) {
-    constexpr int kChunk = kAdamBlock * 4 * V;
     int32_t at = 0;
+    int64_t chunk_at = 0;
     do {
         AdamArgs a;
         const int32_t n = (n_tasks - at) < JMAC_ADAM_MAX_TASKS ? (n_tasks - at) : JMAC_ADAM_MAX_TASKS;
         int64_t chunks = 0;
         for (int32_t i = 0; i < n; ++i) {
             const jmac_adam_task_t& t = tasks[at + i];
-            if (t.n < 0 || (t.n > 0 && (!t.p || !t.g || !t.m || !t.v))) return JMAC_EINVAL;
             a.t[i] = t;
             a.t[i].vec4 = !(((uintptr_t)t.p | (uintptr_t)t.g | (uintptr_t)t.m | (uintptr_t)t.v) & 15);
-            chunks += (t.n + kChunk - 1) / kChunk;
-            if (chunks >= INT32_MAX) return JMAC_ERANGE;
+            chunks += (t.n + kAdamChunk - 1) / kAdamChunk;
             a.chunk_end[i] = (int)chunks;
         }
         for (int32_t i = n; i < JMAC_ADAM_MAX_TASKS; ++i) {
@@ -142,13 +156,20 @@
         a.advance = at >= n_tasks;
         a.step = step;
         a.aux = aux;
-        hipLaunchKernelGGL(adam_step_kernel<V>, dim3((unsigned)(chunks < 1 ? 1 : chunks)), dim3(kAdamBlock), 0, st, a);
+        a.pow = aux + 2 + 2 * chunk_at;
+        chunk_at += chunks;
+        hipLaunchKernelGGL(adam_step_kernel<kAdamV>, dim3((unsigned)(chunks < 1 ? 1 : chunks)), dim3(kAdamBlock), 0, st, a);
         const int rc = (int)hipGetLastError();
         if (rc) return rc;
     } while (at < n_tasks);
     return JMAC_OK;
 }
 
+}
+
+extern "C" int64_t jmac_adam_slots(const jmac_adam_task_t* tasks, int32_t n_tasks) {
+    if (n_tasks < 0 || (n_tasks > 0 && !tasks)) return -1;
+    return adam_chunks(tasks, n_tasks);
 }
 
 extern "C" int jmac_adam_step_f32(const jmac_adam_task_t* tasks, int32_t n_tasks, float* step, double* aux, double lr, double beta1,
@@ -158,6 +179,7 @@
     if (!(lr >= 0.0) || !(eps >= 0.0) || !(beta1 >= 0.0 && beta1 < 1.0) || !(beta2 >= 0.0 && beta2 < 1.0) || !(weight_decay >= 0.0))
         return JMAC_EINVAL;
     for (int32_t i = 0; i < n_tasks; ++i)
-        if (tasks[i].n < 0 || (tasks[i].n > 0 && (!tasks[i].p || !tasks[i].g || !tasks[i].m || !tasks[i].v))) return JMAC_EINVAL;
-    return launch_adam<4>(tasks, n_tasks, step, aux, lr, beta1, beta2, eps, weight_decay, decoupled, maximize, (hipStream_t)stream);
+        if (bad_task(tasks[i])) return JMAC_EINVAL;
+    if (adam_chunks(tasks, n_tasks) < 0) return JMAC_ERANGE;
+    return launch_adam(tasks, n_tasks, step, aux, lr, beta1, beta2, eps, weight_decay, decoupled, maximize, (hipStream_t)stream);
 }
diff --git a/jmac_amd/csrc/scatter.hip b/jmac_amd/csrc/scatter.hip
--- a/jmac_amd/csrc/scatter.hip
+++ b/jmac_amd/csrc/scatter.hip
@@ -111,6 +111,6 @@
     return "jmac: unknown error";
 }
 
-int jmac_version(void) { return 132; }
+int jmac_version(void) { return 133; }
 
 }
diff --git a/jmac_amd/encoder.py b/jmac_amd/encoder.py
--- a/jmac_amd/encoder.py
+++ b/jmac_amd/encoder.py
@@ -110,13 +110,33 @@
         self.c_order = (C.c_int32 * self.nb)(*self.order)
 
 
-def _bn_fwd(x, bn, training, y, y2=None, seg=None, norm=None):
-    use_batch = bool(training or not bn.track_running_stats)
+def _bn_track(bn, training, seg=None):
     if training and bn.track_running_stats:
         if _TRACKERS is not None:
             _TRACKERS.append(bn.num_batches_tracked)
         else:
             bn.num_batches_tracked.add_(seg.nb if seg is not None else 1)
+    return bool(training or not bn.track_running_stats)
+
+
+def _bn_fwd_pair(calls, training, seg=None):
+    paired = (PAIR_LAUNCHES and (seg is None or seg.nb == 1) and
+              all(x.shape[1] <= 512 and bool(training or not bn.track_running_stats) for x, bn, _, _, _ in calls))
+    if not paired:
+        return [_bn_fwd(x, bn, training, y, y2, seg, norm) for x, bn, y, y2, norm in calls]
+    for _, bn, _, _, _ in calls:
+        _bn_track(bn, training, seg)
+    res = ops.bn_tanh_fwd_jobs_raw([(x, bn.weight, bn.bias, bn.running_mean, bn.running_var, bn.momentum, bn.eps, y, y2,
+                                     None if norm is None else (norm.yn, norm.drop, norm.row_map, norm.y_rows))
+                                    for x, bn, y, y2, norm in calls])
+    for (_, _, _, _, norm), (_, _, inv) in zip(calls, res):
+        if norm is not None:
+            norm.inv = inv
+    return [(mean, invstd, True) for mean, invstd, _ in res]
+
+
+def _bn_fwd(x, bn, training, y, y2=None, seg=None, norm=None):
+    use_batch = _bn_track(bn, training, seg)
     if norm is not None:
         mean, invstd, norm.inv = ops.bn_tanh_norm_fwd_raw(x, bn.weight, bn.bias, bn.running_mean, bn.running_var, use_batch,
                                                           bn.momentum, bn.eps, y, norm.yn, norm.drop, norm.row_map, norm.y_rows)
@@ -540,9 +560,9 @@
                            use_batch=use_batch, slope=slope, bn_weight=lay.bn.weight, seg=seg, compact=compact, rows=rows)
 
 
-def _layer_finish(lay, part, agg, training, y, y2=None, seg=None, compact=False, rows=None, norm=None):
+def _layer_finish(lay, part, agg, bn_res, y, seg=None, compact=False, rows=None):
     pre, smax, sden = agg
-    mean, invstd, use_batch = _bn_fwd(pre, lay.bn, training, y, y2, seg, norm)
+    mean, invstd, use_batch = bn_res
     return SimpleNamespace(X=part.X, wc=part.wc, RR=part.RR, a=part.a, PQZ=part.PQZ, pre=pre, smax=smax, sden=sden, y=y, mean=mean,
                            invstd=invstd, use_batch=use_batch, slope=part.slope, bn_weight=lay.bn.weight, seg=seg, compact=compact,
                            rows=rows)
@@ -853,8 +873,10 @@
             pa_ = _layer_fwd(la, align0, t.wc[0], t.cha.RR, a_att[0], graph, training, None, rows=ro, agg=_DEFER)
             pc_ = _layer_fwd(lc, E_n, t.wc[1], t.chc.RR, a_att[1], graph, training, None, rows=ro, agg=_DEFER)
             ra, rc_ = _agg_fwd_pair([(pa_.PQZ, pa_.RR, pa_.a, pa_.slope), (pc_.PQZ, pc_.RR, pc_.a, pc_.slope)], graph, compact=t.rc.on)
-            t.sa = _layer_finish(la, pa_, ra, training, t.catA[:, d:2 * d], t.cat1[:, d:], seg=seg, compact=t.rc.on, rows=ro)
-            t.sc = _layer_finish(lc, pc_, rc_, training, c1, seg=seg, compact=t.rc.on, rows=ro, norm=norm)
+            ba, bc = _bn_fwd_pair([(ra[0], la.bn, t.catA[:, d:2 * d], t.cat1[:, d:], None), (rc_[0], lc.bn, c1, None, norm)], training,
+                                  seg)
+            t.sa = _layer_finish(la, pa_, ra, ba, t.catA[:, d:2 * d], seg=seg, compact=t.rc.on, rows=ro)
+            t.sc = _layer_finish(lc, pc_, rc_, bc, c1, seg=seg, compact=t.rc.on, rows=ro)
         else:
             t.sa = _layer_fwd(la, align0, t.wc[0], t.cha.RR, a_att[0], graph, training, t.catA[:, d:2 * d], t.cat1[:, d:],
                               table_dtype=cfg.table_dtype, seg=seg, compact=t.rc.on, rows=ro)
diff --git a/jmac_amd/ops.py b/jmac_amd/ops.py
--- a/jmac_amd/ops.py
+++ b/jmac_amd/ops.py
@@ -5,7 +5,7 @@
 
 import torch
 
-from ._lib import check, lib, ptr, require_device, stream, testing_lib, workspace
+from ._lib import BnFwdJob, check, lib, ptr, require_device, stream, testing_lib, workspace
 from .graph import RelGraph
 
 BWD_MODE_ATOMIC = 0
@@ -334,6 +334,38 @@
     return mean, invstd, inv
 
 
+def bn_tanh_fwd_jobs_raw(jobs):
+    L = lib()
+    table = (BnFwdJob * len(jobs))()
+    out, keep = [], []
+    for q, (x, weight, bias, running_mean, running_var, momentum, eps, y, y2, norm) in zip(table, jobs):
+        require_device(x, weight, bias, y)
+        N, d = x.shape
+        dev = x.device
+        mean = torch.empty(d, dtype=torch.float32, device=dev)
+        invstd = torch.empty(d, dtype=torch.float32, device=dev)
+        ws_bytes = int(L.jmac_bn_tanh_workspace_bytes(N, d))
+        ws = workspace(ws_bytes, dev)
+        keep.append(ws)
+        q.x, q.ldx, q.N, q.d, q.weight, q.bias = ptr(x), x.stride(0), N, d, ptr(weight), ptr(bias)
+        q.running_mean, q.running_var, q.momentum, q.eps = ptr(running_mean), ptr(running_var), float(momentum), float(eps)
+        q.y, q.ldy, q.save_mean, q.save_invstd, q.ws, q.ws_bytes = ptr(y), y.stride(0), ptr(mean), ptr(invstd), ptr(ws), ws_bytes
+        inv = None
+        if norm is None:
+            q.norm, q.y2, q.ldy2 = 0, ptr(y2), y2.stride(0) if y2 is not None else 0
+        else:
+            if y2 is not None:
+                raise ValueError("bn_tanh_fwd_jobs_raw: the normalise form has no second destination")
+            yn, drop, row_map, y_rows = norm
+            inv = torch.empty(max(N, 1), dtype=torch.float32, device=dev)
+            seed, p_drop = _seed_args(drop)
+            q.norm, q.row_map, q.y_rows, q.ldyr = 1, ptr(row_map), ptr(y_rows), y_rows.stride(0) if y_rows is not None else 0
+            q.norm_eps, q.seed, q.p_drop, q.yn, q.ldyn, q.inv = 1e-12, seed, p_drop, ptr(yn), yn.stride(0), ptr(inv)
+        out.append((mean, invstd, inv))
+    check(L.jmac_bn_tanh_fwd_jobs_f32(table, len(jobs), stream()), "jmac_bn_tanh_fwd_jobs_f32")
+    return out
+
+
 def bn_tanh_bwd_normadj_raw(x, y, inv, drop, g, gy2, row_map, weight, mean, invstd, training: bool):
     L = lib()
     N, d = x.shape
diff --git a/jmac_amd/optim.py b/jmac_amd/optim.py
--- a/jmac_amd/optim.py
+++ b/jmac_amd/optim.py
@@ -23,7 +23,16 @@
 
     @staticmethod
     def _aux(v, betas, dev):
-        return torch.tensor([betas[0] ** v, betas[1] ** v, 0.0], dtype=torch.float64).to(dev)
+        return torch.tensor([betas[0] ** v, betas[1] ** v], dtype=torch.float64).to(dev)
+
+    @staticmethod
+    def _slots(rec, need):
+        if need > rec[4]:
+            if torch.cuda.is_current_stream_capturing():
+                raise RuntimeError("jmac_amd.optim.Adam: the chunks of a step count grew inside a hipGraph capture")
+            rec[2] = rec[2][:2].repeat(1 + need)
+        rec[4] = need
+        return rec[2]
 
     def _counters(self, ps, dev, betas):
         capturing = torch.cuda.is_current_stream_capturing()
@@ -40,7 +49,7 @@
             cn = adopt.get(v)
             if cn is None:
                 cn = adopt[v] = torch.full((), v, dtype=torch.float32, device=dev)
-                self._managed[id(cn)] = [cn, set(), self._aux(v, betas, dev), betas]
+                self._managed[id(cn)] = [cn, set(), self._aux(v, betas, dev), betas, 0]
             self._managed[id(cn)][1].add(id(p))
             st["step"] = cn
         groups = {}
@@ -55,7 +64,7 @@
                     raise RuntimeError("jmac_amd.optim.Adam: the set of parameters with gradients changed inside a hipGraph capture")
                 c2 = c.clone()
                 mine = set(id(p) for p in plist)
-                self._managed[id(c2)] = [c2, mine, self._managed[cid][2].clone(), self._managed[cid][3]]
+                self._managed[id(c2)] = [c2, mine, self._managed[cid][2].clone(), self._managed[cid][3], self._managed[cid][4]]
                 members -= mine
                 for p in plist:
                     self.state[p]["step"] = c2
@@ -64,8 +73,8 @@
             if rec[3] != betas:
                 if capturing:
                     raise RuntimeError("jmac_amd.optim.Adam: betas changed inside a hipGraph capture")
-                rec[2], rec[3] = self._aux(float(c), betas, dev), betas
-            out.append((c, plist, rec[2]))
+                rec[2], rec[3], rec[4] = self._aux(float(c), betas, dev), betas, 0
+            out.append((c, plist, rec))
         return out
 
     def _group_step(self, group):
@@ -86,7 +95,7 @@
                 if st[k].dtype != torch.float32 or not st[k].is_contiguous() or st[k].device != dev:
                     st[k] = st[k].to(device=dev, dtype=torch.float32).contiguous()
         b1, b2 = (float(b) for b in group["betas"])
-        for counter, plist, aux in self._counters(ps, dev, (b1, b2)):
+        for counter, plist, rec in self._counters(ps, dev, (b1, b2)):
             tasks = []
             for p in plist:
                 st = self.state[p]
@@ -98,7 +107,11 @@
                 table = (AdamTask * len(tasks))()
                 for i, (p, g, m, v) in enumerate(tasks):
                     table[i].p, table[i].g, table[i].m, table[i].v, table[i].n, table[i].vec4 = ptr(p), ptr(g), ptr(m), ptr(v), p.numel(), 0
-                cached = self._tables[id(counter)] = (key, table)
+                slots = int(lib().jmac_adam_slots(table, len(tasks)))
+                if slots < 0:
+                    raise ValueError("jmac_amd.optim.Adam: too many parameters for one step count (jmac_adam_slots)")
+                cached = self._tables[id(counter)] = (key, table, slots)
+            aux = self._slots(rec, cached[2])
             check(lib().jmac_adam_step_f32(cached[1], len(tasks), ptr(counter), ptr(aux), float(group["lr"]), b1, b2,
                                            float(group["eps"]), float(group["weight_decay"]), 1 if self._decoupled else 0,
                                            1 if group["maximize"] else 0, stream()), "jmac_adam_step_f32")
```

Result: no change. 31.54 million, median of 6 (+0.9%).
